# microhh/rte-rrtmgp-cpp

Measured on AMD Instinct MI355X. Metric: columns/sec (LW+SW full solve, 140 lay x 256 gpt), higher is better.
Workload: dtype f64; 1 GPU; C4 synthetic 16384 columns/GPU (16384 in total) x 140 layers x 256 g-points, LW+SW clear-sky, RCEMIP profile, synthetic k-distribution (real shapes); columns_per_gpu=16384, columns_total=16384, nlay=140, ngpt=256, flux_mode=broadband (do_broadband solvers, g-point sums on chip), columns_sorted=False, parallelism=columns sharded x1, all-gather of broadband fluxes

## Files before the change

include/rrx_hip.h:

```cpp
#ifndef RRX_HIP_H
#define RRX_HIP_H

#ifdef __cplusplus
extern "C" {
#endif

typedef signed char RrxBool;

const char* rrx_last_error(void);
int rrx_device_count(int* n);
int rrx_set_device(int dev);
int rrx_malloc(void** ptr, unsigned long long bytes);
int rrx_free(void* ptr);
int rrx_malloc_async(void** ptr, unsigned long long bytes, void* stream);
int rrx_free_async(void* ptr, void* stream);
int rrx_free_async_ordered(void* ptr, void* alloc_stream, void* release_stream);
int rrx_memcpy_h2d_stream(void* dst, const void* src, unsigned long long bytes, void* stream);
int rrx_memcpy_d2h_stream(void* dst, const void* src, unsigned long long bytes, void* stream);
int rrx_memcpy_h2d(void* dst, const void* src, unsigned long long bytes);
int rrx_memcpy_d2h(void* dst, const void* src, unsigned long long bytes);
int rrx_memcpy_d2d(void* dst, const void* src, unsigned long long bytes, void* stream);
int rrx_memset(void* dst, int value, unsigned long long bytes, void* stream);
int rrx_synchronize(void* stream);
int rrx_stream_create(void** stream);
// ... 237 lines not shown
        const F* kmajor, const F* kminor_lower, const F* kminor_upper, \
        const int* minor_limits_gpt_lower, const int* minor_limits_gpt_upper, \
        const RrxBool* minor_scales_with_density_lower, const RrxBool* minor_scales_with_density_upper, \
        const RrxBool* scale_by_complement_lower, const RrxBool* scale_by_complement_upper, \
        const int* idx_minor_lower, const int* idx_minor_upper, \
        const int* idx_minor_scaling_lower, const int* idx_minor_scaling_upper, \
        const int* kminor_start_lower, const int* kminor_start_upper, \
        const int* flavor, const F* press_ref_log, const F* temp_ref, \
        F press_ref_log_delta, F temp_ref_min, F temp_ref_delta, F press_ref_trop_log, const F* vmr_ref, \
        const F* play, const F* tlay, const F* tlev, const F* tsfc, int sfc_lay, const F* col_gas, \
        const F* pfracin, F totplnk_delta, const F* totplnk, \
        F* tau, F* pfrac, F* blay, F* blev, F* sfc_src, F* sfc_src_jac, const F* cld_tau, void* stream); \
int rrx_planck_sources_from_fractions##SFX(int ncol, int nlay, int ngpt, const int* gpoint_bands, const F* pfrac, const F* blay, \
        const F* blev, F* lay_src, F* lev_src, void* stream); \
int rrx_lw_solver_noscat_fractions##SFX( \
        int ncol, int nlay, int ngpt, RrxBool top_at_1, const F* secants, const F* weights, \
        const F* tau, const F* pfrac, const F* blay, const F* blev, const int* gpoint_bands, \
        const F* sfc_emis, const F* sfc_src, const F* inc_flux, F* flux_up_loc, F* flux_dn_loc, void* stream); \
 \
int rrx_lw_solver_noscat_fractions_byband##SFX( \
        int ncol, int nlay, int ngpt, int nbnd, RrxBool top_at_1, const F* secants, const F* weights, \
        const F* tau, const F* pfrac, const F* blay, const F* blev, const int* gpoint_bands, const int* band_lims_gpt, \
        const F* sfc_emis, const F* sfc_src, const F* inc_flux, \
        F* bnd_flux_up, F* bnd_flux_dn, F* bnd_flux_net, F* flux_up, F* flux_dn, void* stream); \
 \
int rrx_lw_solver_noscat_fractions_jac##SFX( \
        int ncol, int nlay, int ngpt, RrxBool top_at_1, const F* secants, const F* weights, \
        const F* tau, const F* pfrac, const F* blay, const F* blev, const int* gpoint_bands, \
        const F* sfc_emis, const F* sfc_src, const F* inc_flux, F* flux_up_loc, F* flux_dn_loc, \
        const F* sfc_src_jac, F* flux_up_jac, void* stream); \
 \
int rrx_lw_solver_noscat_fractions_angles##SFX( \
        int ncol, int nlay, int ngpt, RrxBool top_at_1, int nmus, const F* secants, const F* weights, \
        const F* tau, const F* pfrac, const F* blay, const F* blev, const int* gpoint_bands, \
        const F* sfc_emis, const F* sfc_src, const F* inc_flux, F* flux_up_loc, F* flux_dn_loc, \
        const F* sfc_src_jac, F* flux_up_jac, void* stream); \
 \
int rrx_lw_flux_up_adjust##SFX(int ncol, int nlev, const F* flux_up_jac, const F* t_sfc_old, const F* t_sfc_new, \
        F* flux_up, F* flux_net, void* stream); \
 \
int rrx_lw_optimal_secants##SFX(int ncol, int nlay, int ngpt, int nbnd, const int* gpoint_bands, const F* optimal_angle_fit, \
        const F* tau, F* secants, void* stream); \
 \
int rrx_lw_solver_noscat_fractions_optimal##SFX( \
        int ncol, int nlay, int ngpt, int nbnd, RrxBool top_at_1, const F* weights, \
        const F* tau, const F* pfrac, const F* blay, const F* blev, const int* gpoint_bands, const F* optimal_angle_fit, \
        const F* sfc_emis, const F* sfc_src, const F* inc_flux, F* flux_up_loc, F* flux_dn_loc, \
        const F* sfc_src_jac, F* flux_up_jac, F* secants_out, void* stream); \
 \
int rrx_lw_solver_2stream##SFX( \
        int ncol, int nlay, int ngpt, RrxBool top_at_1, \
        const F* tau, const F* ssa, const F* g, const F* lev_source, \
        const F* sfc_emis, const F* sfc_src, const F* inc_flux, \
        F* flux_up, F* flux_dn, RrxBool do_broadband, F* flux_up_loc, F* flux_dn_loc, void* stream); \
 \
int rrx_lw_solver_2stream_fractions##SFX( \
        int ncol, int nlay, int ngpt, int nbnd, RrxBool top_at_1, \
        const F* tau, const F* pfrac, const F* blev, const int* gpoint_bands, const int* band_lims_gpt, \
        const F* cld_tau, const F* cld_ssa, const F* cld_g, \
        const F* sfc_emis, const F* sfc_src, const F* inc_flux, F* flux_up, F* flux_dn, void* stream); \
 \
int rrx_lw_solver_noscat_rescaled##SFX( \
        int ncol, int nlay, int ngpt, RrxBool top_at_1, int nmus, const F* secants, const F* weights, \
        const F* tau, const F* ssa, const F* g, const F* lay_source, const F* lev_source, \
        const F* sfc_emis, const F* sfc_src, const F* inc_flux, F* flux_up, F* flux_dn, \
        RrxBool do_broadband, F* flux_up_loc, F* flux_dn_loc, RrxBool do_jacobians, const F* sfc_src_jac, F* flux_up_jac, void* stream); \
 \
int rrx_lw_solver_noscat_fractions_rescaled##SFX( \
        int ncol, int nlay, int ngpt, int nbnd, RrxBool top_at_1, const F* secants, const F* weights, \
        const F* tau, const F* pfrac, const F* blay, const F* blev, const int* gpoint_bands, const int* band_lims_gpt, \
        const F* cld_tau, const F* cld_ssa, const F* cld_g, \
        const F* sfc_emis, const F* sfc_src, const F* inc_flux, F* flux_up, F* flux_dn, void* stream); \
 \
 \
int rrx_increment_1scalar_by_1scalar##SFX(int ncol, int nlay, int ngpt, F* tau_inout, const F* tau_in, void* stream); \
int rrx_increment_2stream_by_2stream##SFX(int ncol, int nlay, int ngpt, F* tau_inout, F* ssa_inout, F* g_inout, const F* tau_in, const F* ssa_in, const F* g_in, void* stream); \
int rrx_inc_1scalar_by_1scalar_bybnd##SFX(int ncol, int nlay, int ngpt, F* tau_inout, const F* tau_in, int nbnd, const int* band_lims_gpoint, void* stream); \
int rrx_inc_2stream_by_2stream_bybnd##SFX(int ncol, int nlay, int ngpt, F* tau_inout, F* ssa_inout, F* g_inout, const F* tau_in, const F* ssa_in, const F* g_in, int nbnd, const int* band_lims_gpoint, void* stream); \
int rrx_delta_scale_2str_k##SFX(int ncol, int nlay, int ngpt, F* tau_inout, F* ssa_inout, F* g_inout, void* stream); \
 \
int rrx_sum_broadband##SFX(int ncol, int nlev, int ngpt, const F* gpt_flux, F* flux, void* stream); \
int rrx_net_broadband_precalc##SFX(int ncol, int nlev, const F* flux_dn, const F* flux_up, F* flux_net, void* stream); \
 \
int rrx_heating_rate##SFX(int ncol, int nlay, F g_over_cp, const F* flux_net, const F* plev, F* heating_rate, void* stream); \
 \
int rrx_sum_byband##SFX(int ncol, int nlev, int ngpt, int nbnd, const int* band_lims, const F* gpt_flux, F* bnd_flux, void* stream); \
int rrx_net_byband_full##SFX(int ncol, int nlev, int ngpt, int nbnd, const int* band_lims, const F* gpt_flux_dn, const F* gpt_flux_up, F* bnd_flux_net, void* stream); \
 \
int rrx_get_from_subset##SFX(int ncol, int nlay, int nbnd, int ncol_in, int col_s_in, int narr, \
        F* const* var_full, const F* const* var_sub, void* stream); \
 \
 \
int rrx_fill_gases##SFX(int ncol, int nlay, int dim1, int dim2, int ngas, int igas, F* vmr_out, const F* vmr_in, F* col_gas, const F* col_dry, void* stream); \
 \
int rrx_fill_gases_all##SFX(int ncol, int nlay, int ngas, const F* const* vmr_in, const int* dim1, const int* dim2, F* col_gas, const F* col_dry, void* stream); \
 \
int rrx_get_col_dry##SFX(int ncol, int nlay, const F* vmr_h2o, const F* plev, F* col_dry, void* stream); \
 \
int rrx_expand_and_transpose##SFX(int ncol, int nbnd, const int* band_lims_gpt, const F* arr_in, F* arr_out, void* stream); \
 \
int rrx_spread_col##SFX(int ncol, int ngpt, F* toa_src, const F* solar_source, void* stream); \
 \
int rrx_scaling_to_subset##SFX(int ncol, int ngpt, F* toa_src, const F* tsi_scaling, void* stream); \
 \
int rrx_toa_source##SFX(int ncol, int ngpt, F* toa_src, const F* solar_source, const F* tsi_scaling, void* stream); \
 \
int rrx_aerosol_optics##SFX(int ncol, int nlay, int nbnd, int nhum, int nphobic, int nphilic, const F* const* aermr, const int* aermr_per_column, \
        const F* rh, const F* plev, const F* rh_upper, const F* mext_phobic, const F* ssa_phobic, const F* g_phobic, \
        const F* mext_philic, const F* ssa_philic, const F* g_philic, F* tau, F* ssa, F* g, void* stream); \
 \
int rrx_cloud_optics_2str##SFX(int ncol, int nlay, int nbnd, int nsize_liq, int nsize_ice, \
        F radliq_lwr, F radliq_upr, F diamice_lwr, F diamice_upr, \
        const F* lut_extliq, const F* lut_ssaliq, const F* lut_asyliq, \
        const F* lut_extice, const F* lut_ssaice, const F* lut_asyice, \
        const F* clwp, const F* ciwp, const F* reliq, const F* deice, F* tau, F* ssa, F* g, void* stream); \
 \
int rrx_cloud_optics_2str_delta##SFX(int ncol, int nlay, int nbnd, int nsize_liq, int nsize_ice, \
        F radliq_lwr, F radliq_upr, F diamice_lwr, F diamice_upr, \
        const F* lut_extliq, const F* lut_ssaliq, const F* lut_asyliq, \
        const F* lut_extice, const F* lut_ssaice, const F* lut_asyice, \
        const F* clwp, const F* ciwp, const F* reliq, const F* deice, F* tau, F* ssa, F* g, void* stream); \
int rrx_cloud_optics_1scl##SFX(int ncol, int nlay, int nbnd, int nsize_liq, int nsize_ice, \
        F radliq_lwr, F radliq_upr, F diamice_lwr, F diamice_upr, \
        const F* lut_extliq, const F* lut_ssaliq, const F* lut_asyliq, \
        const F* lut_extice, const F* lut_ssaice, const F* lut_asyice, \
        const F* clwp, const F* ciwp, const F* reliq, const F* deice, F* tau, void* stream); \
 \
int rrx_subset_cols##SFX(int ncol_full, int nrest, int col_s, int ncol_sub, const F* in, F* out, void* stream); \
 \
int rrx_subset_lastdim##SFX(int n1, int ncol_full, int col_s, int ncol_sub, const F* in, F* out, void* stream); \
 \
int rrx_fill##SFX(unsigned long long n, F value, F* arr, void* stream); \
 \
int rrx_sort_columns##SFX(int ncol, const F* key, int npad, int* perm, void* stream); \
int rrx_column_spread##SFX(int ncol, const F* key, int block, F threshold, int* flag, void* stream); \
int rrx_gather_cols##SFX(int nout, unsigned long long nrest, const int* perm, int ncol_in, const F* in, F* out, void* stream); \
int rrx_scatter_cols##SFX(int n, unsigned long long nrest, const int* perm, int ncol_src, const F* in, int ncol_dst, F* out, void* stream); \
int rrx_gather_lastdim##SFX(int n1, int nout, const int* perm, const F* in, F* out, void* stream); \
 \
int rrx_sunlit_columns##SFX(int ncol, const F* mu0, const int* order, int pad_to, int* perm, int* count, void* stream); \
int rrx_scatter_cols_fill##SFX(int n, unsigned long long nrest, const int* perm, int ncol_src, const F* in, int ncol_dst, F* out, void* stream); \
 \
int rrx_mcica_increment_1scalar##SFX(int ncol, int nlay, int ngpt, int nbnd, const int* band_lims_gpt, const F* cloud_frac, const F* alpha, \
        unsigned long long seed, int domain, const int* col_id, int col_id0, F* tau_inout, const F* cld_tau, unsigned char* mask_out, void* stream); \
int rrx_mcica_increment_2stream##SFX(int ncol, int nlay, int ngpt, int nbnd, const int* band_lims_gpt, const F* cloud_frac, const F* alpha, \
        unsigned long long seed, int domain, const int* col_id, int col_id0, F* tau_inout, F* ssa_inout, F* g_inout, \
        const F* cld_tau, const F* cld_ssa, const F* cld_g, unsigned char* mask_out, void* stream); \
int rrx_mcica_cloud_mask##SFX(int ncol, int nlay, int ngpt, const F* cloud_frac, const F* alpha, unsigned long long seed, int domain, \
        const int* col_id, int col_id0, unsigned char* mask_out, void* stream); \
 \
int rrx_rt_k_null##SFX(int nx, int ny, int nz, int ngpt, int nbnd, int igpt, RrxBool top_at_1, const F* tau, const int* band_lims_gpt, \
        const F* cld_tau, F dz, int knx, int kny, int knz, F* k_null, void* stream); \
int rrx_rt_trace_counts##SFX(int nx, int ny, int nz, int ngpt, int nbnd, int igpt, RrxBool top_at_1, RrxBool independent_column, \
        const F* tau, const F* ssa, const int* band_lims_gpt, const F* cld_tau, const F* cld_ssa, const F* cld_g, \
        F dx, F dy, F dz, const F* sfc_albedo, F mu0, F azimuth, F inc_dir, F inc_dif, int knx, int kny, int knz, const F* k_null, \
        unsigned long long seed, long long photon0, long long nphotons, int max_events, \
        unsigned long long* sfc_dn_dir, unsigned long long* sfc_dn_dif, unsigned long long* sfc_up, unsigned long long* tod_up, \
        unsigned long long* abs_dir, unsigned long long* abs_dif, unsigned long long* n_capped, void* stream); \
int rrx_rt_counts_to_flux##SFX(long long n, const unsigned long long* counts, F scale, F* out, void* stream); \
int rrx_raytracer_sw##SFX(int nx, int ny, int nz, int ngpt, int nbnd, RrxBool top_at_1, RrxBool independent_column, \
        const F* tau, const F* ssa, const int* band_lims_gpt, const F* cld_tau, const F* cld_ssa, const F* cld_g, \
        F dx, F dy, F dz, const F* sfc_albedo, F mu0, F azimuth, const F* inc_dir, const F* inc_dif, int knx, int kny, int knz, \
        long long photons_per_pixel, unsigned long long seed, int max_events, \
        F* sfc_dn_dir, F* sfc_dn_dif, F* sfc_up, F* tod_up, F* abs_dir, F* abs_dif, unsigned long long* n_capped, void* stream); \
 \
int rrx_rt_bw_trace_counts##SFX(int nx, int ny, int nz, int ngpt, int nbnd, int igpt, RrxBool top_at_1, \
        const F* tau, const F* ssa, const int* band_lims_gpt, const F* cld_tau, const F* cld_ssa, const F* cld_g, \
        F dx, F dy, F dz, const F* sfc_albedo, F mu0, F azimuth, int knx, int kny, int knz, const F* k_null, \
        int sensor_type, int npx, int npy, F fov, const F* sensor, unsigned long long seed, long long ray0, long long nrays, int max_events, \
        unsigned long long* counts, unsigned long long* n_capped, unsigned long long* n_clamped, void* stream); \
int rrx_raytracer_bw##SFX(int nx, int ny, int nz, int ngpt, int nbnd, RrxBool top_at_1, \
        const F* tau, const F* ssa, const int* band_lims_gpt, const F* cld_tau, const F* cld_ssa, const F* cld_g, \
        F dx, F dy, F dz, const F* sfc_albedo, F mu0, F azimuth, const F* inc_dir, int knx, int kny, int knz, \
        int sensor_type, int npx, int npy, F fov, const F* sensor, long long rays_per_pixel, unsigned long long seed, int max_events, \
        F* radiance, unsigned long long* n_capped, unsigned long long* n_clamped, void* stream);

RRX_DECLARE(double, _f64)
RRX_DECLARE(float, _f32)

#ifdef __cplusplus
}
#endif
#endif
```

rte-rrtmgp-cpp_amd/csrc/rrx_common.h:

```cpp
#ifndef RRX_COMMON_H
#define RRX_COMMON_H

#include <hip/hip_runtime.h>
#include <cfloat>
#include <cstdlib>
#include <cmath>
#include <string>
#include <vector>
#include <stdexcept>
#include <type_traits>
#include <initializer_list>
#include <utility>
#include "rrx_hip.h"

typedef signed char Bool;

namespace rrx
{
    struct Tuning
    {
        int lw_variant = 0;
        int sw_variant = 0;
        int bb_min_groups = 512;
        int bb_gsplit = 0;
// ... 108 lines not shown
#else
    __device__ __forceinline__ float fast_rcp(const float x) { return 1.0f / x; }
#endif

    __device__ __forceinline__ double exp_neg(const double x)
    {
        const double n = __builtin_rint(x * 0x1.71547652b82fep+0);
        double r = fma(n, -0x1.62e42f0000000p-1, x);
        r = fma(n, -0x1.df473de6af279p-26, r);
        double p = 0x1.af389ecfc4b9cp-26;
        p = fma(p, r, 0x1.28917c89a43a7p-22); p = fma(p, r, 0x1.71de0db2f6b19p-19); p = fma(p, r, 0x1.a019b9149a41cp-16);
        p = fma(p, r, 0x1.a01a01a7c2efep-13); p = fma(p, r, 0x1.6c16c17889ef1p-10); p = fma(p, r, 0x1.11111111109b5p-7);
        p = fma(p, r, 0x1.5555555553d68p-5); p = fma(p, r, 0x1.5555555555556p-3); p = fma(p, r, 0x1.0000000000001p-1);
        const double t = fma(r*r, p, r);
        return __builtin_amdgcn_ldexp(t + 1.0, (int)n);
    }
    static __device__ const double exp2_64_table[64] = {
        0x1.0000000000000p+0, 0x1.02c9a3e778061p+0, 0x1.059b0d3158574p+0, 0x1.0874518759bc8p+0, 0x1.0b5586cf9890fp+0, 0x1.0e3ec32d3d1a2p+0,
        0x1.11301d0125b51p+0, 0x1.1429aaea92de0p+0, 0x1.172b83c7d517bp+0, 0x1.1a35beb6fcb75p+0, 0x1.1d4873168b9aap+0, 0x1.2063b88628cd6p+0,
        0x1.2387a6e756238p+0, 0x1.26b4565e27cddp+0, 0x1.29e9df51fdee1p+0, 0x1.2d285a6e4030bp+0, 0x1.306fe0a31b715p+0, 0x1.33c08b26416ffp+0,
        0x1.371a7373aa9cbp+0, 0x1.3a7db34e59ff7p+0, 0x1.3dea64c123422p+0, 0x1.4160a21f72e2ap+0, 0x1.44e086061892dp+0, 0x1.486a2b5c13cd0p+0,
        0x1.4bfdad5362a27p+0, 0x1.4f9b2769d2ca7p+0, 0x1.5342b569d4f82p+0, 0x1.56f4736b527dap+0, 0x1.5ab07dd485429p+0, 0x1.5e76f15ad2148p+0,
        0x1.6247eb03a5585p+0, 0x1.6623882552225p+0, 0x1.6a09e667f3bcdp+0, 0x1.6dfb23c651a2fp+0, 0x1.71f75e8ec5f74p+0, 0x1.75feb564267c9p+0,
        0x1.7a11473eb0187p+0, 0x1.7e2f336cf4e62p+0, 0x1.82589994cce13p+0, 0x1.868d99b4492edp+0, 0x1.8ace5422aa0dbp+0, 0x1.8f1ae99157736p+0,
        0x1.93737b0cdc5e5p+0, 0x1.97d829fde4e50p+0, 0x1.9c49182a3f090p+0, 0x1.a0c667b5de565p+0, 0x1.a5503b23e255dp+0, 0x1.a9e6b5579fdbfp+0,
        0x1.ae89f995ad3adp+0, 0x1.b33a2b84f15fbp+0, 0x1.b7f76f2fb5e47p+0, 0x1.bcc1e904bc1d2p+0, 0x1.c199bdd85529cp+0, 0x1.c67f12e57d14bp+0,
        0x1.cb720dcef9069p+0, 0x1.d072d4a07897cp+0, 0x1.d5818dcfba487p+0, 0x1.da9e603db3285p+0, 0x1.dfc97337b9b5fp+0, 0x1.e502ee78b3ff6p+0,
        0x1.ea4afa2a490dap+0, 0x1.efa1bee615a27p+0, 0x1.f50765b6e4540p+0, 0x1.fa7c1819e90d8p+0};
    __device__ __forceinline__ void exp_table_fill(double* lds_table)
    {
        if (threadIdx.x < 64) lds_table[threadIdx.x] = exp2_64_table[threadIdx.x];
    }
    __device__ __forceinline__ double exp_neg(const double x, const double* lds_table)
    {
        const double magic = 0x1.8p+52;
        const double t = fma(x, 0x1.71547652b82fep+6, magic);
        const double nf = t - magic;
        double r = fma(nf, -0x1.62e42fefa0000p-7, x);
        r = fma(nf, -0x1.cf79abc9e3b3ap-46, r);
        const int j = __double2loint(t) & 63;
        const int e = ((int)nf >> 6);
        const double T = lds_table[j];
        double p = 0x1.1111111111111p-7;
        p = fma(p, r, 0x1.5555555555555p-5); p = fma(p, r, 0x1.5555555555555p-3); p = fma(p, r, 0.5);
        const double q = fma(r*r, p, r);
        return __builtin_amdgcn_ldexp(fma(T, q, T), e);
    }
    __device__ __forceinline__ float exp_neg(const float x)
    {
        const float p = x * 0x1.715476p+0f;
        const float d = fmaf(x, 0x1.4ae0c0p-26f, fmaf(x, 0x1.715476p+0f, -p));
        const float y = __builtin_amdgcn_exp2f(p);
        return fmaf(y, d * 0x1.62e430p-1f, y);
    }
    __device__ __forceinline__ float exp_neg(const float x, const float*) { return exp_neg(x); }

    __device__ __forceinline__ double sqrt_pos(const double x)
    {
        const double y = __builtin_amdgcn_rsq(x);
        double g = x*y, h = 0.5*y;
        const double r = fma(-h, g, 0.5);
        g = fma(g, r, g); h = fma(h, r, h);
        const double d = fma(-g, g, x);
        return fma(d, h, g);
    }
    __device__ __forceinline__ float sqrt_pos(const float x) { return __builtin_amdgcn_sqrtf(x); }

    __device__ __forceinline__ double sqrt_nonneg(const double x)
    {
        const double y = __builtin_fmin(__builtin_amdgcn_rsq(x), 0x1p+511);
        double g = x*y, h = 0.5*y;
        const double r = fma(-h, g, 0.5);
        g = fma(g, r, g); h = fma(h, r, h);
        const double d = fma(-g, g, x);
        return fma(d, h, g);
    }
    __device__ __forceinline__ float sqrt_nonneg(const float x) { return sqrt_pos(x); }

    __device__ __forceinline__ int xcd_contiguous(const int w, const int n)
    {
        constexpr int NXCD = 8;
        const int per = n / NXCD, whole = per*NXCD;
        return (w < whole) ? (w % NXCD)*per + w / NXCD : w;
    }

    inline int ceil_div(const long long a, const long long b) { return int((a + b - 1) / b); }

    template<typename Fn> void with_flag(const bool flag, Fn&& f) { if (flag) f(std::true_type{}); else f(std::false_type{}); }

    template<int... Ks, typename Fn> bool with_k(const int need, Fn&& f)
    {
        return ((need <= Ks && (f(std::integral_constant<int,Ks>{}), true)) || ...);
    }

    inline void keep_pool_memory()
    {
        static thread_local int configured_device = -1;
        int dev = 0;
        if (hipGetDevice(&dev) != hipSuccess || dev == configured_device) return;
        hipMemPool_t pool;
        if (hipDeviceGetDefaultMemPool(&pool, dev) != hipSuccess) return;
        unsigned long long keep = ~0ull;
        if (const char* e = std::getenv("RRX_POOL_RELEASE_THRESHOLD")) keep = std::strtoull(e, nullptr, 10);
        if (hipMemPoolSetAttribute(pool, hipMemPoolAttrReleaseThreshold, &keep) == hipSuccess) configured_device = dev;
    }

    void* cached_workspace(hipStream_t st, size_t bytes);
    void release_workspace(hipStream_t st);
    void trim_workspace(hipStream_t st);
    size_t workspace_bytes(hipStream_t st);

    class WorkspaceLease
    {
        public:
            explicit WorkspaceLease(hipStream_t st) : st_(st) {}
            WorkspaceLease(const WorkspaceLease&) = delete;
            WorkspaceLease& operator=(const WorkspaceLease&) = delete;
            template<typename F> F* get(const size_t n)
            {
                if (taken_) throw std::runtime_error("workspace leased twice in one call");
                taken_ = true;
                return static_cast<F*>(cached_workspace(st_, n*sizeof(F)));
            }
            ~WorkspaceLease() { if (taken_) trim_workspace(st_); }
        private:
            hipStream_t st_;
            bool taken_ = false;
    };

    class StreamScratch
    {
        public:
            explicit StreamScratch(hipStream_t st) : st_(st) {}
            StreamScratch(const StreamScratch&) = delete;
            StreamScratch& operator=(const StreamScratch&) = delete;
            template<typename F> F* get(const size_t n, const bool zero = false)
            {
                void* p = nullptr;
                keep_pool_memory();
                if (hipMallocAsync(&p, n*sizeof(F), st_) != hipSuccess) throw std::runtime_error("workspace allocation failed");
                ptrs_.push_back(p);
                if (zero && hipMemsetAsync(p, 0, n*sizeof(F), st_) != hipSuccess) throw std::runtime_error("workspace memset failed");
                return static_cast<F*>(p);
            }
            ~StreamScratch() { for (void* p : ptrs_) (void)hipFreeAsync(p, st_); }
        private:
            hipStream_t st_;
            std::vector<void*> ptrs_;
    };
}

namespace rrx
{
    inline int broadband_gsplit(const int groups, const int ngpt, const int slots = 512)
    {
        const Tuning& t = tuning();
        if (t.bb_gsplit >= 1) return std::min(t.bb_gsplit, ngpt);
        if (t.bb_min_groups <= 1) return 1;
        int best = 1;
        double best_cost = double(ceil_div(groups, slots));
        for (int n = 2, k = 1; n <= 16 && n*4 <= ngpt; n *= 2, ++k)
        {
            const double cost = double(ceil_div((long long)groups*n, slots)) / n * (1.0 + 0.01*k);
            if (cost < best_cost) { best_cost = cost; best = n; }
        }
        return best;
// ... 154 lines not shown
```

rte-rrtmgp-cpp_amd/csrc/rrx_gas_optics.hip:

```cpp
#include <type_traits>
#include <cstdio>
#include <cstdlib>
#include "rrx_common.h"
#include "rrx_hip.h"

namespace
{
#ifndef RRX_GW_ABL
#define RRX_GW_ABL 0
#endif
template<typename F> __device__ __forceinline__ void stream_store_sbase(const char* sbase, const unsigned voff, const F v)
{
    static_assert(sizeof(F) == 4 || sizeof(F) == 8, "dword or dwordx2");
    if (RRX_GW_ABL == 7) { if (v == F(-12345.678)) *reinterpret_cast<F*>(const_cast<char*>(sbase) + voff) = v; return; }
    if constexpr (sizeof(F) == 4) asm volatile("global_store_dword %0, %1, %2 nt" :: "v"(voff), "v"(v), "s"(sbase) : "memory");
    else asm volatile("global_store_dwordx2 %0, %1, %2 nt" :: "v"(voff), "v"(v), "s"(sbase) : "memory");
}
template<typename F> __device__ __forceinline__ void stream_store(F* p, const F v)
{
    if (RRX_GW_ABL == 7) { if (v == F(-12345.678)) *p = v; return; }
    __builtin_nontemporal_store(v, p);
}

using namespace rrx;
// ... 1110 lines not shown
{
    if (const char* e = std::getenv("RRX_GW_GEOM")) return std::atoi(e) ? 1 : 0;
    return ncol >= 192 ? 1 : 0;
}
inline dim3 gather_grid(const int entries_)
{
    const int entries = entries_*GSH;
    return dim3(std::min(entries, 512));
}
inline dim3 gas_window_grid(const int geom, const int ncol, const int nlay)
{
    return geom ? dim3(ceil_div(ncol, 256), nlay) : dim3(ceil_div(ncol, 64), ceil_div(nlay, 4));
}

#ifndef RRX_GW_TIMING
#define RRX_GW_TIMING 0
#endif
#if RRX_GW_TIMING
__device__ unsigned long long g_gw_clk[8];
#define RRX_GW_T(k) { const unsigned long long t_ = __builtin_readcyclecounter(); gw_acc[k] += t_ - gw_t; gw_t = t_; }
#else
#define RRX_GW_T(k)
#endif
thread_local long long g_gw_handed = 0, g_gw_total = 0;
inline void gas_window_stats(const char* what, const int* todo, const int nblk, hipStream_t st)
{
    if (std::getenv("RRX_GW_STATS") == nullptr) return;
    int h[9];
    if (hipStreamSynchronize(st) != hipSuccess || hipMemcpy(h, todo - 8, sizeof(h), hipMemcpyDeviceToHost) != hipSuccess) return;
    g_gw_handed += h[8]; g_gw_total += nblk;
    std::fprintf(stderr, "[gas window %s] %d of %d workgroups handed back: temperature %d, pressure %d, regimes %d, chunk form %d, eta %d\n",
                 what, h[8], nblk, h[0], h[1], h[2], h[3], h[4]);
#if RRX_GW_TIMING
    unsigned long long clk[8], zero[8] = {0};
    if (hipMemcpyFromSymbol(clk, HIP_SYMBOL(g_gw_clk), sizeof(clk)) == hipSuccess)
    {
        std::fprintf(stderr, "[gas window %s] clocks per workgroup (wavefront 0): set-up %.0f, chunk prologue %.0f, staging %.0f, dma wait %.0f, barriers %.0f, g-point loop %.0f, tail %.0f, contributor scalings %.0f\n",
                     what, double(clk[0])/nblk, double(clk[1])/nblk, double(clk[2])/nblk, double(clk[3])/nblk, double(clk[4])/nblk, double(clk[5])/nblk, double(clk[6])/nblk, double(clk[7])/nblk);
        (void)hipMemcpyToSymbol(HIP_SYMBOL(g_gw_clk), zero, sizeof(zero));
    }
#endif
}

template<typename F> struct PlanckArgs
{
    const F* pfracin; const F* tlev; const F* tsfc; int sfc_lay; int nPlanckTemp; const int* gpoint_bands;
    F totplnk_delta; const F* totplnk; F* pfrac; F* blay; F* blev; F* sfc_src; F* sfc_src_jac;
};

struct GasWindowTables
{
    int ngpt, nmax, ncmax;
    static constexpr int LIT = 1 + NXW;
    __host__ __device__ int off_cinfo() const { return 2*ngpt; }
    __host__ __device__ int off_lists() const { return off_cinfo() + ncmax + 3; }
    __host__ __device__ int off_mmeta() const { return off_lists() + 2*ncmax*LIT; }
    __host__ __device__ int off_cuni()  const { return off_mmeta() + 2*MM*nmax; }
    __host__ __device__ int off_order() const { return off_cuni() + 2*ncmax; }
    static constexpr int GX = 6;
    static constexpr int RH = 12;
    static constexpr int RC = 8;
    static constexpr int REC = RH + RC*NXW;
    __host__ __device__ int off_gx()    const { return (off_order() + 2*ncmax + 3) & ~3; }
    __host__ __device__ int off_bad()   const { return off_gx() + GX*ngpt; }
    __host__ __device__ int off_rec()   const { return (off_bad() + 2*(ncmax + 1) + 3) & ~3; }
    __host__ __device__ int ints()      const { return off_rec() + 2*ncmax*REC; }
};
static_assert(GasWindowTables::REC % 4 == 0 && GasWindowTables::RH % 4 == 0 && GasWindowTables::RC == 8, "records are read as 16- and 32-byte words");
inline int gas_window_ncmax(const int ngpt, const int nband) { return (ngpt + GCH - 1) / GCH + std::max(nband, 0); }

constexpr int GW_TBL_HEADER = 8;
constexpr int GW_TBL_MAGIC = 0x52525835;
__global__ void __launch_bounds__(256)
gas_window_tables_kernel(
        const int ngpt, const int nminorlower, const int nminorupper, const int ncmax, const int nlist, const int nband,
        const int* __restrict__ gpoint_flavor,
        const int* __restrict__ flavor, const int* __restrict__ gpoint_bands, const int* __restrict__ band_lims,
        const int* __restrict__ minor_limits_gpt_lower, const int* __restrict__ minor_limits_gpt_upper,
        const Bool* __restrict__ minor_scales_with_density_lower, const Bool* __restrict__ minor_scales_with_density_upper,
        const Bool* __restrict__ scale_by_complement_lower, const Bool* __restrict__ scale_by_complement_upper,
        const int* __restrict__ idx_minor_lower, const int* __restrict__ idx_minor_upper,
        const int* __restrict__ idx_minor_scaling_lower, const int* __restrict__ idx_minor_scaling_upper,
        const int* __restrict__ kminor_start_lower, const int* __restrict__ kminor_start_upper,
        int* __restrict__ tbl)
{
    extern __shared__ int lds_int[];
    const int nmax = max(nminorlower, nminorupper);
    const GasWindowTables T{ngpt, nmax, ncmax};
    constexpr int LIT = GasWindowTables::LIT;
    int* gflav = lds_int;
    int* cinfo = lds_int + T.off_cinfo();
    int* lists = lds_int + T.off_lists();
    int* mmeta = lds_int + T.off_mmeta();
    int* cuni = lds_int + T.off_cuni();
    int* order = lds_int + T.off_order();
    int* cut = lds_int + T.off_gx();
    const int tid = threadIdx.x;
    const int ntab = T.off_gx();
    auto gx_of = [&](const int g, const int k) -> int
    {
        if (k == 0) return gpoint_bands != nullptr ? gpoint_bands[g] - 1 : -1;
        if (k == 1)
        {
            if (band_lims == nullptr) return -1;
            int b = 0;
            while (b < nband-1 && g + 1 > band_lims[2*b+1]) ++b;
            return b;
        }
        return flavor[2*gflav[((k - 2) >> 1)*ngpt + g] + (k & 1)];
    };
    for (int w = tid; w < ntab + ngpt + 4 + 2*((ngpt + 63)/64); w += 256) lds_int[w] = 0;
    __syncthreads();
    {
        for (int w = tid; w < 2*ngpt; w += 256) gflav[(w & 1)*ngpt + (w >> 1)] = gpoint_flavor[w] - 1;
        for (int w = tid; w < nminorlower; w += 256)
        {
            int* m = mmeta + MM*w;
            m[0] = idx_minor_lower[w]; m[1] = minor_scales_with_density_lower[w] ? 1 : 0;
            m[2] = idx_minor_scaling_lower[w]; m[3] = scale_by_complement_lower[w] ? 1 : 0;
            m[4] = minor_limits_gpt_lower[2*w]; m[5] = minor_limits_gpt_lower[2*w+1]; m[6] = kminor_start_lower[w];
        }
        for (int w = tid; w < nminorupper; w += 256)
        {
            int* m = mmeta + MM*(nmax + w);
            m[0] = idx_minor_upper[w]; m[1] = minor_scales_with_density_upper[w] ? 1 : 0;
            m[2] = idx_minor_scaling_upper[w]; m[3] = scale_by_complement_upper[w] ? 1 : 0;
            m[4] = minor_limits_gpt_upper[2*w]; m[5] = minor_limits_gpt_upper[2*w+1]; m[6] = kminor_start_upper[w];
        }
    }
    __syncthreads();
    {
        int* head = tbl + T.ints();
        int differs = (head[0] != GW_TBL_MAGIC || head[1] != ngpt || head[2] != nminorlower || head[3] != nminorupper
                       || head[4] != ncmax || head[5] != nlist || head[6] != nband) ? 1 : 0;
        for (int w = tid; w < 2*ngpt && !differs; w += 256) differs = (tbl[w] != gflav[w]) ? 1 : 0;
        for (int w = tid; w < 2*MM*nmax && !differs; w += 256) differs = (tbl[T.off_mmeta() + w] != mmeta[w]) ? 1 : 0;
        for (int w = tid; w < GasWindowTables::GX*ngpt && !differs; w += 256)
            differs = (tbl[T.off_gx() + w] != gx_of(w / GasWindowTables::GX, w % GasWindowTables::GX)) ? 1 : 0;
        if (!__syncthreads_or(differs)) return;
        if (tid == 0) head[0] = 0;
    }
    for (int g = tid; g < ngpt; g += 256)
        if (g > 0 && (gflav[g] != gflav[g-1] || gflav[ngpt + g] != gflav[ngpt + g-1])) cut[g] = 1;
    for (int w = tid; w < 2*nmax; w += 256)
    {
        const int r = w / nmax, i = w % nmax;
        if (i < (r == 0 ? nminorlower : nminorupper))
        {
            const int* m = mmeta + MM*w;
            const int lo = m[4]-1, hi = m[5];
            if (lo > 0 && lo < ngpt) cut[lo] = 1;
            if (hi > 0 && hi < ngpt) cut[hi] = 1;
        }
    }
    __syncthreads();
    unsigned long long* cutmask = reinterpret_cast<unsigned long long*>(cut + ((ngpt + 2) & ~1));
    for (int base = 0; base < ngpt; base += 256)
    {
        const int g = base + tid;
        const unsigned long long m = __ballot(g > 0 && g < ngpt && cut[g] != 0);
        if ((tid & 63) == 0 && base + (tid & ~63) < ngpt) cutmask[(base + tid) >> 6] = m;
    }
    __syncthreads();
    if (tid == 0)
    {
        int n = 0, start = 0;
        bool fits = true;
        auto emit_until = [&](const int p)
        {
// ... 779 lines not shown

template<typename F> size_t planck_lds_bytes(const int ngpt)
{
    return size_t(GCH)*(PL+1)*64*sizeof(F) + size_t((2*ngpt + 3) & ~3)*sizeof(int) + size_t(PL)*2*4*GCH*2*sizeof(F);
}


template<typename F>
struct GasTables
{
    int nband, ngpt, neta, npres, ntemp, nminorlower, nminorupper, idx_h2o;
    const int* gpoint_flavor; const int* band_lims_gpt;
    const F* kmajor; const F* kminor_lower; const F* kminor_upper;
    const int* minor_limits_gpt_lower; const int* minor_limits_gpt_upper;
    const Bool* minor_scales_with_density_lower; const Bool* minor_scales_with_density_upper;
    const Bool* scale_by_complement_lower; const Bool* scale_by_complement_upper;
    const int* idx_minor_lower; const int* idx_minor_upper;
    const int* idx_minor_scaling_lower; const int* idx_minor_scaling_upper;
    const int* kminor_start_lower; const int* kminor_start_upper;
    const F* krayl = nullptr;
};

template<typename F>
struct GasCells
{
    int ncol, nlay;
    const F* play; const F* tlay; const F* col_gas; const F* col_dry = nullptr; F* tau = nullptr; F* ssa = nullptr; F* g = nullptr;
    const Bool* tropo = nullptr; const F* col_mix = nullptr; const F* fmajor = nullptr; const F* fminor = nullptr;
    const int* jeta = nullptr; const int* jtemp = nullptr; const int* jpress = nullptr;
};

struct TodoTail { const int* todo = nullptr; int gx = 1, nblk = 1, nz = 1, geom = 0; };

inline size_t gather_lds_bytes(const int ngpt, const int nminorlower, const int nminorupper)
{
    const int nchunk = (ngpt + GCH - 1) / GCH, nmax = std::max(nminorlower, nminorupper);
    const size_t lds = (size_t(3)*ngpt + size_t(2)*nchunk*(1 + ITEM*nmax) + size_t(2)*MM*nmax)*sizeof(int);
    if (lds > 64*1024) throw std::runtime_error("minor-gas index exceeds 64 KiB of LDS");
    return lds;
}

template<typename F, int MODE, bool DIRECT, bool CLD>
void launch_tau_absorption(hipStream_t st, const dim3 grid, const size_t lds, const GasTables<F>& k, const GasCells<F>& c, const InterpArgs<F>& ia,
                           const TodoTail& t = TodoTail())
{
    tau_absorption_kernel<F,MODE,DIRECT,CLD><<<grid, dim3(64, 4), lds, st>>>(
            c.ncol, c.nlay, k.ngpt, k.neta, k.npres, k.ntemp, k.nminorlower, k.nminorupper, k.idx_h2o, k.gpoint_flavor,
            k.kmajor, k.kminor_lower, k.kminor_upper, k.minor_limits_gpt_lower, k.minor_limits_gpt_upper,
            k.minor_scales_with_density_lower, k.minor_scales_with_density_upper,
            k.scale_by_complement_lower, k.scale_by_complement_upper,
            k.idx_minor_lower, k.idx_minor_upper, k.idx_minor_scaling_lower, k.idx_minor_scaling_upper,
            k.kminor_start_lower, k.kminor_start_upper,
            c.tropo, c.col_mix, c.fmajor, c.fminor, c.play, c.tlay, c.col_gas, c.col_dry, c.jeta, c.jtemp, c.jpress, k.krayl,
            c.tau, c.ssa, c.g, ia, t.todo, t.gx, t.nblk, t.nz, t.geom);
}

struct GasWindowPlan
{
    bool windowed = false;
    int geom = 0, nblk = 0, nz = 1, ncmax = 0;
    dim3 grid;
    size_t lds = 0;
    int* todo = nullptr; int* tbl = nullptr;
    TodoTail tail() const { return windowed ? TodoTail{todo, int(grid.x), nblk, nz, geom} : TodoTail(); }
};

template<typename F>
GasWindowPlan gas_window_plan(hipStream_t st, StreamScratch& scratch, const GasTables<F>& k, const GasCells<F>& c, const InterpArgs<F>& ia,
                              const int mode, const bool pf, const int nlist, const int* gpoint_bands)
{
    GasWindowPlan p;
    const int nchunk = (k.ngpt + GCH - 1) / GCH;
    const int nmax = std::max(k.nminorlower, k.nminorupper);
    p.ncmax = gas_window_ncmax(k.ngpt, k.nband);
    p.lds = gas_window_lds_bytes<F>(k.ngpt, nmax, p.ncmax, mode, pf);
    p.windowed = tuning().go_window && p.lds <= 64*1024 && size_t(c.ncol)*c.nlay*sizeof(F) < (size_t(1) << 32)
                 && size_t(k.ngpt)*k.ntemp*k.neta*(k.npres+1)*sizeof(F) < (size_t(1) << 32);
    if (!p.windowed) return p;
    p.geom = gas_window_geometry(c.ncol);
    p.grid = gas_window_grid(p.geom, c.ncol, c.nlay);
    p.nblk = int(p.grid.x)*int(p.grid.y);
    p.nz = gas_window_parts(p.nblk, nchunk);
    p.todo = scratch.get<int>(size_t(9) + size_t(p.nblk)*p.nz) + 8;
    if (hipMemsetAsync(p.todo - 8, 0, 9*sizeof(int), st) != hipSuccess) throw std::runtime_error("memset failed");
    const GasWindowTables T{k.ngpt, nmax, p.ncmax};
    const int* lims = ia.cld_tau != nullptr ? ia.cld_lims : nullptr;
    p.tbl = gas_window_tables(st, k.gpoint_flavor, k.ngpt, k.nminorlower, k.nminorupper, p.ncmax, nlist, (pf ? 1 : 0) + (lims != nullptr ? 2 : 0));
    gas_window_tables_kernel<<<1, 256, size_t(T.off_gx() + k.ngpt + 4 + 2*((k.ngpt + 63)/64))*sizeof(int), st>>>(
            k.ngpt, k.nminorlower, k.nminorupper, p.ncmax, nlist, k.nband, k.gpoint_flavor, ia.flavor, gpoint_bands, lims,
            k.minor_limits_gpt_lower, k.minor_limits_gpt_upper,
            k.minor_scales_with_density_lower, k.minor_scales_with_density_upper, k.scale_by_complement_lower, k.scale_by_complement_upper,
            k.idx_minor_lower, k.idx_minor_upper, k.idx_minor_scaling_lower, k.idx_minor_scaling_upper,
            k.kminor_start_lower, k.kminor_start_upper, p.tbl);
    return p;
}

template<typename F, int MODE, bool PF, bool CLD>
void launch_gas_window(hipStream_t st, const GasWindowPlan& p, const GasTables<F>& k, const GasCells<F>& c, const InterpArgs<F>& ia,
                       const PlanckArgs<F>& pa = PlanckArgs<F>())
{
    gas_window_kernel<F,MODE,PF,CLD><<<dim3(p.grid.x, p.grid.y, p.nz), dim3(64, 4), p.lds, st>>>(
            c.ncol, c.nlay, k.ngpt, k.neta, k.npres, k.ntemp, k.nminorlower, k.nminorupper, k.idx_h2o, k.gpoint_flavor,
            k.kmajor, k.kminor_lower, k.kminor_upper, k.minor_limits_gpt_lower, k.minor_limits_gpt_upper,
            k.minor_scales_with_density_lower, k.minor_scales_with_density_upper,
            k.scale_by_complement_lower, k.scale_by_complement_upper,
            k.idx_minor_lower, k.idx_minor_upper, k.idx_minor_scaling_lower, k.idx_minor_scaling_upper,
            k.kminor_start_lower, k.kminor_start_upper, c.play, c.tlay, c.col_gas, c.col_dry, k.krayl, ia,
            c.tau, c.ssa, c.g, pa, p.todo, p.geom, p.tbl, p.ncmax);
}

template<bool ALLOWED, typename F, typename Fn>
void with_cld(const InterpArgs<F>& ia, Fn&& fn)
{
    if constexpr (ALLOWED) { if (ia.cld_tau != nullptr) { fn(std::bool_constant<true>{}); return; } }
    fn(std::bool_constant<false>{});
}

template<typename F>
int gas_optics_lw_fractions_impl(const GasTables<F>& k, const GasCells<F>& c, const InterpArgs<F>& ia, const PlanckArgs<F>& pa, void* stream)
{
    RRX_TRY
    if (c.ncol <= 0 || c.nlay <= 0 || k.ngpt <= 0) throw std::runtime_error("empty problem");
    hipStream_t st = static_cast<hipStream_t>(stream);
    const size_t lds = gather_lds_bytes(k.ngpt, k.nminorlower, k.nminorupper);
    StreamScratch scratch(st);
    const GasWindowPlan p = gas_window_plan<F>(st, scratch, k, c, ia, 2, true, NXW, pa.gpoint_bands);
    const dim3 g2 = p.windowed ? gather_grid(p.nblk*p.nz) : dim3(ceil_div(c.ncol, 64), ceil_div(c.nlay, 4));
    const TodoTail t = p.tail();
    with_cld<true>(ia, [&](auto CLD_)
    {
        constexpr bool CLD = decltype(CLD_)::value;
        if (p.windowed)
        {
            launch_gas_window<F,2,true,CLD>(st, p, k, c, ia, pa);
            gas_window_stats("lw + fractions", p.todo, p.nblk*p.nz, st);
        }
        launch_tau_absorption<F,2,true,CLD>(st, g2, lds, k, c, ia, t);
    });
    planck_fraction_kernel<F><<<g2, dim3(64, 4), size_t(2)*k.ngpt*sizeof(int), st>>>(
            c.ncol, c.nlay, k.ngpt, k.neta, k.npres, k.ntemp, pa.nPlanckTemp, c.play, c.tlay, pa.tlev, pa.tsfc, pa.sfc_lay, c.col_gas, ia,
            pa.gpoint_bands, pa.pfracin, pa.totplnk_delta, pa.totplnk, k.gpoint_flavor, pa.pfrac, pa.blay, pa.blev, pa.sfc_src, pa.sfc_src_jac,
            t.todo, t.gx, t.nblk, t.nz, t.geom);
    RRX_CATCH("rrx_gas_optics_lw_fractions")
}

template<typename F, int MODE, bool DIRECT = false>
int tau_absorption_impl(const GasTables<F>& k, const GasCells<F>& c, void* stream, const char* name, const InterpArgs<F>& ia = InterpArgs<F>())
{
    RRX_TRY
    if (c.ncol <= 0 || c.nlay <= 0 || k.ngpt <= 0) throw std::runtime_error("empty problem");
    hipStream_t st = static_cast<hipStream_t>(stream);
    const size_t lds = gather_lds_bytes(k.ngpt, k.nminorlower, k.nminorupper);
    constexpr bool HAS_CLD = DIRECT && MODE != 0;
    StreamScratch scratch(st);
    GasWindowPlan p;
    if constexpr (DIRECT && MODE != 0) p = gas_window_plan<F>(st, scratch, k, c, ia, MODE, false, (MODE == 1) ? NCW : NXW, nullptr);
    with_cld<HAS_CLD>(ia, [&](auto CLD_)
    {
        constexpr bool CLD = decltype(CLD_)::value;
        if constexpr (DIRECT && MODE != 0)
        {
            if (p.windowed)
            {
                launch_gas_window<F,MODE,false,CLD>(st, p, k, c, ia);
                gas_window_stats(MODE == 1 ? "sw" : "lw", p.todo, p.nblk*p.nz, st);
                launch_tau_absorption<F,MODE,DIRECT,CLD>(st, gather_grid(p.nblk*p.nz), lds, k, c, ia, p.tail());
                return;
            }
        }
        launch_tau_absorption<F,MODE,DIRECT,CLD>(st, dim3(ceil_div(c.ncol, 64), ceil_div(c.nlay, 4)), lds, k, c, ia);
    });
    RRX_CATCH(name)
}
}


// ... 332 lines not shown
```

rte-rrtmgp-cpp_amd/csrc/rrx_misc.hip:

```cpp
#include <mutex>
#include <vector>
#include <cstdlib>
#include <initializer_list>
#include "rrx_common.h"
#include "rrx_hip.h"

namespace rrx
{
    static thread_local std::string g_last_error;
    void set_error(const std::string& msg) { g_last_error = msg; }
    Tuning& tuning()
    {
        static thread_local Tuning t = []
        {
            Tuning d;
            if (const char* e = getenv("RRX_SYNC")) d.sync_waves = atoi(e);
            if (const char* e = getenv("RRX_GO_SHARE")) d.go_share = atoi(e);
            if (const char* e = getenv("RRX_GO_WINDOW")) d.go_window = atoi(e);
            return d;
        }();
        return t;
    }
    namespace
    {
// ... 90 lines not shown
{
    RRX_GRID_STRIDE(i, n) tau1[i] = tau1[i] + tau2[i];
}

template<typename F>
__device__ __forceinline__ void inc_2str(F& tau1, F& ssa1, F& g1, const F tau2, const F ssa2, const F g2, const F eps)
{
    const F tau12 = tau1 + tau2;
    const F tauscat12 = (tau1 * ssa1) + (tau2 * ssa2);
    g1 = ((tau1 * ssa1 * g1) + (tau2 * ssa2 * g2)) / max(tauscat12, eps);
    ssa1 = tauscat12 / max(eps, tau12);
    tau1 = tau12;
}

template<typename F>
__global__ void inc_2str_kernel(const size_t n, const F eps, F* __restrict__ tau1, F* __restrict__ ssa1, F* __restrict__ g1,
        const F* __restrict__ tau2, const F* __restrict__ ssa2, const F* __restrict__ g2)
{
    RRX_GRID_STRIDE(i, n)
    {
        F t = tau1[i], w = ssa1[i], gg = g1[i];
        inc_2str(t, w, gg, tau2[i], ssa2[i], g2[i], eps);
        tau1[i] = t; ssa1[i] = w; g1[i] = gg;
    }
}

template<typename F>
__global__ void inc_1scl_bybnd_kernel(const size_t ncl, F* __restrict__ tau1, const F* __restrict__ tau2,
        const int nbnd, const int* __restrict__ band_lims_gpt)
{
    const int igpt = blockIdx.y;
    for (int ibnd=0; ibnd<nbnd; ++ibnd)
        if (igpt+1 >= band_lims_gpt[2*ibnd] && igpt+1 <= band_lims_gpt[2*ibnd+1])
        {
            RRX_GRID_STRIDE(i, ncl) tau1[i + igpt*ncl] = tau1[i + igpt*ncl] + tau2[i + ibnd*ncl];
        }
}

template<typename F>
__global__ void inc_2str_bybnd_kernel(const size_t ncl, const F eps, F* __restrict__ tau1, F* __restrict__ ssa1, F* __restrict__ g1,
        const F* __restrict__ tau2, const F* __restrict__ ssa2, const F* __restrict__ g2,
        const int nbnd, const int* __restrict__ band_lims_gpt)
{
    const int igpt = blockIdx.y;
    for (int ibnd=0; ibnd<nbnd; ++ibnd)
        if (igpt+1 >= band_lims_gpt[2*ibnd] && igpt+1 <= band_lims_gpt[2*ibnd+1])
        {
            RRX_GRID_STRIDE(i, ncl)
            {
                const size_t o = i + igpt*ncl, b = i + ibnd*ncl;
                F t = tau1[o], w = ssa1[o], gg = g1[o];
                inc_2str(t, w, gg, tau2[b], ssa2[b], g2[b], eps);
                tau1[o] = t; ssa1[o] = w; g1[o] = gg;
            }
        }
}

template<typename F>
__global__ void delta_scale_kernel(const size_t n, const F eps, F* __restrict__ tau, F* __restrict__ ssa, F* __restrict__ g)
{
    RRX_GRID_STRIDE(i, n)
    {
        const F gv = g[i], wv = ssa[i];
        const F f = gv * gv;
        const F wf = wv * f;
        tau[i] *= (F(1.) - wf);
        ssa[i] = (wv - wf) / max(eps, F(1.) - wf);
        g[i] = (gv - f) / max(eps, F(1.) - f);
    }
}

template<typename F>
__global__ void sum_broadband_kernel(const size_t nlc, const int ngpt, const F* __restrict__ in, F* __restrict__ out)
{
    RRX_GRID_STRIDE(i, nlc)
    {
        F s = F(0.);
        for (int ig=0; ig<ngpt; ++ig) s += in[i + size_t(ig)*nlc];
        out[i] = s;
    }
}

template<typename F>
__global__ void net_kernel(const size_t n, const F* __restrict__ dn, const F* __restrict__ up, F* __restrict__ net)
{
    RRX_GRID_STRIDE(i, n) net[i] = dn[i] - up[i];
}

template<typename F, bool NET>
__global__ void byband_kernel(const size_t nlc, const int* __restrict__ band_lims, const F* __restrict__ a, const F* __restrict__ b, F* __restrict__ out)
{
    const int ibnd = blockIdx.y;
    const int g0 = band_lims[2*ibnd]-1, g1 = band_lims[2*ibnd+1]-1;
    if (g1 < g0)
    {
        RRX_GRID_STRIDE(i, nlc) out[i + size_t(ibnd)*nlc] = F(0.);
        return;
    }
    RRX_GRID_STRIDE(i, nlc)
    {
        F s = NET ? a[i + size_t(g0)*nlc] - b[i + size_t(g0)*nlc] : a[i + size_t(g0)*nlc];
        for (int ig=g0+1; ig<=g1; ++ig)
            s += NET ? a[i + size_t(ig)*nlc] - b[i + size_t(ig)*nlc] : a[i + size_t(ig)*nlc];
        out[i + size_t(ibnd)*nlc] = s;
    }
}

template<typename F> struct PtrPack { F* full[4]; const F* sub[4]; };

template<typename F>
__global__ void get_from_subset_kernel(const int ncol, const size_t nrest, const int ncol_in, const int col_s_in, const int narr, const PtrPack<F> p)
{
    const size_t n = size_t(ncol_in)*nrest;
    RRX_GRID_STRIDE(i, n)
    {
        const size_t ic = i % ncol_in, r = i / ncol_in;
        const size_t o = ic + col_s_in - 1 + r*ncol;
        for (int a=0; a<narr; ++a) p.full[a][o] = p.sub[a][i];
    }
}

template<typename F>
__global__ void fill_gases_kernel(const int ncol, const int nlay, const int dim1, const int dim2, const int igas,
        F* __restrict__ vmr_out, const F* __restrict__ vmr_in, F* __restrict__ col_gas, const F* __restrict__ col_dry)
{
    const size_t ncl = size_t(ncol)*nlay;
    RRX_GRID_STRIDE(i, ncl)
    {
        if (igas > 0)
        {
            F v;
            if (dim1 == 1 && dim2 == 1) v = vmr_in[0];
            else if (dim1 == 1)         v = vmr_in[i / ncol];
            else                        v = vmr_in[i];
            vmr_out[i + size_t(igas-1)*ncl] = v;
            col_gas[i + size_t(igas)*ncl] = v * col_dry[i];
        }
        else
            col_gas[i] = col_dry[i];
    }
}

constexpr int RRX_MAX_GASES = 32;
template<typename F> struct GasTable { const F* vmr[RRX_MAX_GASES]; int dim1[RRX_MAX_GASES], dim2[RRX_MAX_GASES]; };

template<typename F>
__global__ void fill_gases_all_kernel(const int ncol, const int nlay, const int ngas, const GasTable<F> gt,
                                      F* __restrict__ col_gas, const F* __restrict__ col_dry)
{
    const size_t ncl = size_t(ncol)*nlay;
    RRX_GRID_STRIDE(i, ncl)
    {
        const F cd = col_dry[i];
        col_gas[i] = cd;
        for (int igas=0; igas<ngas; ++igas)
        {
            const F* __restrict__ src = gt.vmr[igas];
            const F v = (gt.dim1[igas] == 1 && gt.dim2[igas] == 1) ? src[0] : (gt.dim1[igas] == 1 ? src[i / ncol] : src[i]);
            col_gas[i + size_t(igas+1)*ncl] = v * cd;
        }
    }
}

template<typename F>
__global__ void col_dry_kernel(const int ncol, const int nlay, const F* __restrict__ vmr_h2o, const F* __restrict__ plev, F* __restrict__ col_dry)
{
    constexpr F g0 = 9.80665;
    constexpr F avogad = 6.02214076e23;
    constexpr F m_dry = 0.028964;
    constexpr F m_h2o = 0.018016;
    const size_t ncl = size_t(ncol)*nlay;
    RRX_GRID_STRIDE(i, ncl)
    {
        const F delta_plev = abs(plev[i] - plev[i + ncol]);
        const F h = vmr_h2o[i];
        const F m_air = (m_dry + m_h2o * h) / (F(1.) + h);
        F cd = F(10.) * delta_plev * avogad / (F(1000.)*m_air*F(100.)*g0);
        cd /= (F(1.) + h);
        col_dry[i] = cd;
    }
}

template<typename F>
__global__ void expand_and_transpose_kernel(const int ncol, const int nbnd, const int* __restrict__ limits, const F* __restrict__ in, F* __restrict__ out)
{
    const int ibnd = blockIdx.y;
    const int g0 = limits[2*ibnd]-1, g1 = limits[2*ibnd+1];
    RRX_GRID_STRIDE(icol, size_t(ncol))
    {
        const F v = in[ibnd + icol*nbnd];
        for (int ig=g0; ig<g1; ++ig) out[icol + size_t(ig)*ncol] = v;
    }
}

template<typename F>
__global__ void spread_col_kernel(const int ncol, const int ngpt, F* __restrict__ out, const F* __restrict__ src)
{
    const F v = src[blockIdx.y];
    for (int icol = blockIdx.x*blockDim.x + threadIdx.x; icol < ncol; icol += gridDim.x*blockDim.x) out[icol + size_t(blockIdx.y)*ncol] = v;
}

template<typename F>
__global__ void scale_cols_kernel(const int ncol, const int ngpt, F* __restrict__ out, const F* __restrict__ fac)
{
    for (int icol = blockIdx.x*blockDim.x + threadIdx.x; icol < ncol; icol += gridDim.x*blockDim.x) out[icol + size_t(blockIdx.y)*ncol] *= fac[icol];
}

template<typename F>
__global__ void toa_source_kernel(const int ncol, const int ngpt, F* __restrict__ out, const F* __restrict__ src, const F* __restrict__ fac)
{
    const F v = src[blockIdx.y];
    for (int icol = blockIdx.x*blockDim.x + threadIdx.x; icol < ncol; icol += gridDim.x*blockDim.x) out[icol + size_t(blockIdx.y)*ncol] = v * fac[icol];
}

template<typename F>
__device__ __forceinline__ void cloud_from_table(const F cwp, const F re, const int nsteps, const F step_size, const F offset,
        const F* __restrict__ tau_table, const F* __restrict__ ssa_table, const F* __restrict__ asy_table,
        F& tau, F& taussa, F& taussag)
{
    if (cwp > F(0.))
    {
        const int index = min(int((re - offset) / step_size)+1, nsteps-1);
        const F fint = (re - offset) / step_size - (index-1);
        tau = cwp * (tau_table[index-1] + fint * (tau_table[index] - tau_table[index-1]));
        taussa = tau * (ssa_table[index-1] + fint * (ssa_table[index] - ssa_table[index-1]));
        taussag = taussa * (asy_table[index-1] + fint * (asy_table[index] - asy_table[index-1]));
    }
    else { tau = F(0.); taussa = F(0.); taussag = F(0.); }
}

template<typename F, bool TWOSTR, bool DELTA>
__global__ void cloud_optics_kernel(const size_t ncl, const int nbnd, const int nsize_liq, const int nsize_ice,
        const F radliq_lwr, const F liq_step, const F diamice_lwr, const F ice_step,
        const F* __restrict__ lut_extliq, const F* __restrict__ lut_ssaliq, const F* __restrict__ lut_asyliq,
        const F* __restrict__ lut_extice, const F* __restrict__ lut_ssaice, const F* __restrict__ lut_asyice,
        const F* __restrict__ clwp, const F* __restrict__ ciwp, const F* __restrict__ reliq, const F* __restrict__ deice,
        F* __restrict__ tau, F* __restrict__ ssa, F* __restrict__ g)
{
    const F eps = Lim<F>::eps();
    const F eps_delta = Lim<F>::tiny()*F(3.);
    RRX_GRID_STRIDE(i, ncl)
    {
        const F lw = clwp[i], iw = ciwp[i], rl = reliq[i], di = deice[i];
        int il = 1, ii = 1; F fl = F(0.), fi = F(0.);
        if (lw > F(0.)) { il = min(int((rl - radliq_lwr) / liq_step)+1, nsize_liq-1); fl = (rl - radliq_lwr) / liq_step - (il-1); }
        if (iw > F(0.)) { ii = min(int((di - diamice_lwr) / ice_step)+1, nsize_ice-1); fi = (di - diamice_lwr) / ice_step - (ii-1); }
        for (int ibnd=0; ibnd<nbnd; ++ibnd)
        {
            F lt = F(0.), lts = F(0.), ltsg = F(0.), it = F(0.), its = F(0.), itsg = F(0.);
            if (lw > F(0.))
            {
                const F* te = lut_extliq + size_t(ibnd)*nsize_liq; const F* ts = lut_ssaliq + size_t(ibnd)*nsize_liq; const F* ta = lut_asyliq + size_t(ibnd)*nsize_liq;
                lt = lw * (te[il-1] + fl * (te[il] - te[il-1]));
                lts = lt * (ts[il-1] + fl * (ts[il] - ts[il-1]));
                ltsg = lts * (ta[il-1] + fl * (ta[il] - ta[il-1]));
            }
            if (iw > F(0.))
            {
                const F* te = lut_extice + size_t(ibnd)*nsize_ice; const F* ts = lut_ssaice + size_t(ibnd)*nsize_ice; const F* ta = lut_asyice + size_t(ibnd)*nsize_ice;
                it = iw * (te[ii-1] + fi * (te[ii] - te[ii-1]));
                its = it * (ts[ii-1] + fi * (ts[ii] - ts[ii-1]));
                itsg = its * (ta[ii-1] + fi * (ta[ii] - ta[ii-1]));
            }
            const size_t o = i + size_t(ibnd)*ncl;
            if constexpr (TWOSTR)
            {
                const F t = lt + it, tsc = lts + its, tsg = ltsg + itsg;
                F tv = t, wv = tsc / max(t, eps), gv = tsg / max(tsc, eps);
                if constexpr (DELTA)
                {
                    const F f = gv * gv;
                    const F wf = wv * f;
                    tv *= (F(1.) - wf);
                    const F w2 = (wv - wf) / max(eps_delta, F(1.) - wf);
                    gv = (gv - f) / max(eps_delta, F(1.) - f);
                    wv = w2;
                }
                tau[o] = tv; ssa[o] = wv; g[o] = gv;
            }
            else
                tau[o] = (lt - lts) + (it - its);
        }
    }
}

template<typename F> struct AerosolSpecies { const F* mmr[11]; int per_column[11]; };

__constant__ const signed char aerosol_species_table[11][3] = {
    {0, 1, 0}, {1, 1, 1}, {2, 1, 2},
    {3, 0, 0}, {4, 0, 7}, {5, 0, 5},
    {7, 0, 9}, {6, 1, 3},
    {8, 0, 10}, {9, 0, 10},
    {10, 1, 4}};

template<typename F>
// ... 111 lines not shown
        hipEvent_t ev;
        ok = hipEventCreateWithFlags(&ev, hipEventDisableTiming) == hipSuccess;
        if (ok)
        {
            ok = hipEventRecord(ev, a) == hipSuccess && hipStreamWaitEvent(r, ev, 0) == hipSuccess;
            (void)hipEventDestroy(ev);
        }
    }
    if (ok && hipFreeAsync(ptr, r) == hipSuccess) return 0;
    (void)hipGetLastError();
    RRX_HIP_OK(hipFree(ptr), "rrx_free_async_ordered");
    return 0;
}
int rrx_memcpy_h2d_stream(void* dst, const void* src, unsigned long long bytes, void* stream)
{
    RRX_HIP_OK(hipMemcpyAsync(dst, src, bytes, hipMemcpyHostToDevice, static_cast<hipStream_t>(stream)), "rrx_memcpy_h2d_stream");
    RRX_HIP_OK(hipStreamSynchronize(static_cast<hipStream_t>(stream)), "rrx_memcpy_h2d_stream");
    return 0;
}
int rrx_memcpy_d2h_stream(void* dst, const void* src, unsigned long long bytes, void* stream)
{
    RRX_HIP_OK(hipMemcpyAsync(dst, src, bytes, hipMemcpyDeviceToHost, static_cast<hipStream_t>(stream)), "rrx_memcpy_d2h_stream");
    RRX_HIP_OK(hipStreamSynchronize(static_cast<hipStream_t>(stream)), "rrx_memcpy_d2h_stream");
    return 0;
}
int rrx_memcpy_h2d(void* dst, const void* src, unsigned long long bytes) { RRX_HIP_OK(hipMemcpy(dst, src, bytes, hipMemcpyHostToDevice), "rrx_memcpy_h2d"); return 0; }
int rrx_memcpy_d2h(void* dst, const void* src, unsigned long long bytes) { RRX_HIP_OK(hipMemcpy(dst, src, bytes, hipMemcpyDeviceToHost), "rrx_memcpy_d2h"); return 0; }
int rrx_memcpy_d2d(void* dst, const void* src, unsigned long long bytes, void* stream) { RRX_HIP_OK(hipMemcpyAsync(dst, src, bytes, hipMemcpyDeviceToDevice, static_cast<hipStream_t>(stream)), "rrx_memcpy_d2d"); return 0; }
int rrx_memset(void* dst, int value, unsigned long long bytes, void* stream) { RRX_HIP_OK(hipMemsetAsync(dst, value, bytes, static_cast<hipStream_t>(stream)), "rrx_memset"); return 0; }
int rrx_synchronize(void* stream) { RRX_HIP_OK(hipStreamSynchronize(static_cast<hipStream_t>(stream)), "rrx_synchronize"); return 0; }
int rrx_stream_create(void** stream) { hipStream_t s; RRX_HIP_OK(hipStreamCreate(&s), "rrx_stream_create"); *stream = s; return 0; }
int rrx_stream_destroy(void* stream)
{
    rrx::release_workspace(static_cast<hipStream_t>(stream));
    RRX_HIP_OK(hipStreamDestroy(static_cast<hipStream_t>(stream)), "rrx_stream_destroy");
    return 0;
}
int rrx_release_workspace(void* stream) { rrx::release_workspace(static_cast<hipStream_t>(stream)); return 0; }
unsigned long long rrx_workspace_bytes(void* stream) { return rrx::workspace_bytes(static_cast<hipStream_t>(stream)); }

#define ST static_cast<hipStream_t>(stream)

int rrx_subset_nd(void* out, const void* in, int elem_bytes, int ndim, const int* sub_dims, const long long* strides,
                  const int* starts, const int* spread, void* stream)
{
    RRX_TRY
    if (ndim < 1 || ndim > 7) throw std::runtime_error("ndim must be 1..7");
    if (elem_bytes != 1 && elem_bytes != 4 && elem_bytes != 8) throw std::runtime_error("element size must be 1, 4 or 8 bytes");
    SubsetND sd; sd.ndim = ndim; size_t n = 1;
    for (int d=0; d<ndim; ++d)
    {
        if (sub_dims[d] < 0) throw std::runtime_error("negative extent");
        sd.sub_dims[d] = sub_dims[d]; sd.strides[d] = strides[d]; sd.starts[d] = starts[d]; sd.spread[d] = spread[d]; n *= size_t(sub_dims[d]);
    }
    if (n == 0) return 0;
    if (elem_bytes == 8) subset_nd_kernel<double><<<grid1d(n), 256, 0, ST>>>(sd, n, static_cast<const double*>(in), static_cast<double*>(out));
    else if (elem_bytes == 4) subset_nd_kernel<int><<<grid1d(n), 256, 0, ST>>>(sd, n, static_cast<const int*>(in), static_cast<int*>(out));
    else subset_nd_kernel<signed char><<<grid1d(n), 256, 0, ST>>>(sd, n, static_cast<const signed char*>(in), static_cast<signed char*>(out));
    RRX_CATCH("rrx_subset_nd")
}

#define RRX_DEFINE_MISC(F, SFX) \
int rrx_increment_1scalar_by_1scalar##SFX(int ncol, int nlay, int ngpt, F* tau_inout, const F* tau_in, void* stream) \
{ RRX_TRY const size_t n = size_t(ncol)*nlay*ngpt; \
  inc_1scl_kernel<F><<<grid1d(n), 256, 0, ST>>>(n, tau_inout, tau_in); RRX_CATCH("rrx_increment_1scalar_by_1scalar") } \
int rrx_increment_2stream_by_2stream##SFX(int ncol, int nlay, int ngpt, F* tau_inout, F* ssa_inout, F* g_inout, const F* tau_in, const F* ssa_in, const F* g_in, void* stream) \
{ RRX_TRY const size_t n = size_t(ncol)*nlay*ngpt; \
  inc_2str_kernel<F><<<grid1d(n), 256, 0, ST>>>(n, rrx::Lim<F>::tiny()*F(3.), tau_inout, ssa_inout, g_inout, tau_in, ssa_in, g_in); RRX_CATCH("rrx_increment_2stream_by_2stream") } \
int rrx_inc_1scalar_by_1scalar_bybnd##SFX(int ncol, int nlay, int ngpt, F* tau_inout, const F* tau_in, int nbnd, const int* band_lims_gpoint, void* stream) \
{ RRX_TRY const size_t ncl = extent({ncol, nlay}); if (extent({ngpt, nbnd}) == 0 || ncl == 0) return 0; \
  inc_1scl_bybnd_kernel<F><<<dim3(std::min(grid1d(ncl), 1024), ngpt), 256, 0, ST>>>(ncl, tau_inout, tau_in, nbnd, band_lims_gpoint); RRX_CATCH("rrx_inc_1scalar_by_1scalar_bybnd") } \
int rrx_inc_2stream_by_2stream_bybnd##SFX(int ncol, int nlay, int ngpt, F* tau_inout, F* ssa_inout, F* g_inout, const F* tau_in, const F* ssa_in, const F* g_in, int nbnd, const int* band_lims_gpoint, void* stream) \
{ RRX_TRY const size_t ncl = extent({ncol, nlay}); if (extent({ngpt, nbnd}) == 0 || ncl == 0) return 0; \
  inc_2str_bybnd_kernel<F><<<dim3(std::min(grid1d(ncl), 1024), ngpt), 256, 0, ST>>>(ncl, rrx::Lim<F>::tiny()*F(3.), tau_inout, ssa_inout, g_inout, tau_in, ssa_in, g_in, nbnd, band_lims_gpoint); RRX_CATCH("rrx_inc_2stream_by_2stream_bybnd") } \
int rrx_delta_scale_2str_k##SFX(int ncol, int nlay, int ngpt, F* tau_inout, F* ssa_inout, F* g_inout, void* stream) \
{ RRX_TRY const size_t n = size_t(ncol)*nlay*ngpt; \
  delta_scale_kernel<F><<<grid1d(n), 256, 0, ST>>>(n, rrx::Lim<F>::tiny()*F(3.), tau_inout, ssa_inout, g_inout); RRX_CATCH("rrx_delta_scale_2str_k") } \
int rrx_sum_broadband##SFX(int ncol, int nlev, int ngpt, const F* gpt_flux, F* flux, void* stream) \
{ RRX_TRY const size_t n = size_t(ncol)*nlev; \
  sum_broadband_kernel<F><<<grid1d(n), 256, 0, ST>>>(n, ngpt, gpt_flux, flux); RRX_CATCH("rrx_sum_broadband") } \
int rrx_net_broadband_precalc##SFX(int ncol, int nlev, const F* flux_dn, const F* flux_up, F* flux_net, void* stream) \
{ RRX_TRY const size_t n = size_t(ncol)*nlev; \
  net_kernel<F><<<grid1d(n), 256, 0, ST>>>(n, flux_dn, flux_up, flux_net); RRX_CATCH("rrx_net_broadband_precalc") } \
int rrx_heating_rate##SFX(int ncol, int nlay, F g_over_cp, const F* flux_net, const F* plev, F* heating_rate, void* stream) \
{ RRX_TRY const size_t n = extent({ncol, nlay}); if (n == 0) return 0; \
  heating_rate_kernel<F><<<grid1d(n), 256, 0, ST>>>(n, ncol, g_over_cp, flux_net, plev, heating_rate); RRX_CATCH("rrx_heating_rate") } \
int rrx_sum_byband##SFX(int ncol, int nlev, int ngpt, int nbnd, const int* band_lims, const F* gpt_flux, F* bnd_flux, void* stream) \
{ RRX_TRY (void)ngpt; const size_t n = extent({ncol, nlev}); if (n == 0 || extent({nbnd}) == 0) return 0; \
  byband_kernel<F,false><<<dim3(std::min(grid1d(n), 1024), nbnd), 256, 0, ST>>>(n, band_lims, gpt_flux, (const F*)nullptr, bnd_flux); RRX_CATCH("rrx_sum_byband") } \
int rrx_net_byband_full##SFX(int ncol, int nlev, int ngpt, int nbnd, const int* band_lims, const F* gpt_flux_dn, const F* gpt_flux_up, F* bnd_flux_net, void* stream) \
{ RRX_TRY (void)ngpt; const size_t n = extent({ncol, nlev}); if (n == 0 || extent({nbnd}) == 0) return 0; \
  byband_kernel<F,true><<<dim3(std::min(grid1d(n), 1024), nbnd), 256, 0, ST>>>(n, band_lims, gpt_flux_dn, gpt_flux_up, bnd_flux_net); RRX_CATCH("rrx_net_byband_full") } \
int rrx_get_from_subset##SFX(int ncol, int nlay, int nbnd, int ncol_in, int col_s_in, int narr, F* const* var_full, const F* const* var_sub, void* stream) \
{ RRX_TRY if (narr < 1 || narr > 4) throw std::runtime_error("narr must be 1..4"); \
  if (col_s_in < 1 || col_s_in - 1 + ncol_in > ncol) throw std::runtime_error("column range outside the full array"); \
  PtrPack<F> p; for (int a=0; a<narr; ++a) { p.full[a] = var_full[a]; p.sub[a] = var_sub[a]; } \
  const size_t nrest = extent({nlay, nbnd}); if (extent({ncol_in}) == 0 || nrest == 0) return 0; \
  get_from_subset_kernel<F><<<grid1d(size_t(ncol_in)*nrest), 256, 0, ST>>>(ncol, nrest, ncol_in, col_s_in, narr, p); RRX_CATCH("rrx_get_from_subset") } \
int rrx_fill_gases##SFX(int ncol, int nlay, int dim1, int dim2, int ngas, int igas, F* vmr_out, const F* vmr_in, F* col_gas, const F* col_dry, void* stream) \
{ RRX_TRY (void)ngas; if (extent({ncol, nlay}) == 0) return 0; \
  fill_gases_kernel<F><<<grid1d(size_t(ncol)*nlay), 256, 0, ST>>>(ncol, nlay, dim1, dim2, igas, vmr_out, vmr_in, col_gas, col_dry); RRX_CATCH("rrx_fill_gases") } \
int rrx_fill_gases_all##SFX(int ncol, int nlay, int ngas, const F* const* vmr_in, const int* dim1, const int* dim2, F* col_gas, const F* col_dry, void* stream) \
{ RRX_TRY if (ngas < 0 || ngas > RRX_MAX_GASES) throw std::runtime_error("more gases than rrx_fill_gases_all takes"); \
  if (extent({ncol, nlay}) == 0) return 0; \
  GasTable<F> gt; for (int i=0; i<ngas; ++i) { gt.vmr[i] = vmr_in[i]; gt.dim1[i] = dim1[i]; gt.dim2[i] = dim2[i]; } \
  fill_gases_all_kernel<F><<<grid1d(size_t(ncol)*nlay), 256, 0, ST>>>(ncol, nlay, ngas, gt, col_gas, col_dry); RRX_CATCH("rrx_fill_gases_all") } \
int rrx_get_col_dry##SFX(int ncol, int nlay, const F* vmr_h2o, const F* plev, F* col_dry, void* stream) \
{ RRX_TRY col_dry_kernel<F><<<grid1d(size_t(ncol)*nlay), 256, 0, ST>>>(ncol, nlay, vmr_h2o, plev, col_dry); RRX_CATCH("rrx_get_col_dry") } \
int rrx_expand_and_transpose##SFX(int ncol, int nbnd, const int* band_lims_gpt, const F* arr_in, F* arr_out, void* stream) \
{ RRX_TRY if (extent({ncol, nbnd}) == 0) return 0; \
  expand_and_transpose_kernel<F><<<dim3(std::min(grid1d(ncol), 1024), nbnd), 256, 0, ST>>>(ncol, nbnd, band_lims_gpt, arr_in, arr_out); RRX_CATCH("rrx_expand_and_transpose") } \
int rrx_spread_col##SFX(int ncol, int ngpt, F* toa_src, const F* solar_source, void* stream) \
{ RRX_TRY spread_col_kernel<F><<<dim3(std::min(ceil_div(ncol, 256), 64), ngpt), 256, 0, ST>>>(ncol, ngpt, toa_src, solar_source); RRX_CATCH("rrx_spread_col") } \
int rrx_scaling_to_subset##SFX(int ncol, int ngpt, F* toa_src, const F* tsi_scaling, void* stream) \
{ RRX_TRY scale_cols_kernel<F><<<dim3(std::min(ceil_div(ncol, 256), 64), ngpt), 256, 0, ST>>>(ncol, ngpt, toa_src, tsi_scaling); RRX_CATCH("rrx_scaling_to_subset") } \
int rrx_toa_source##SFX(int ncol, int ngpt, F* toa_src, const F* solar_source, const F* tsi_scaling, void* stream) \
{ RRX_TRY if (ncol <= 0 || ngpt <= 0) throw std::runtime_error("empty problem"); \
  if (tsi_scaling == nullptr) spread_col_kernel<F><<<dim3(std::min(ceil_div(ncol, 256), 64), ngpt), 256, 0, ST>>>(ncol, ngpt, toa_src, solar_source); \
  else toa_source_kernel<F><<<dim3(std::min(ceil_div(ncol, 256), 64), ngpt), 256, 0, ST>>>(ncol, ngpt, toa_src, solar_source, tsi_scaling); RRX_CATCH("rrx_toa_source") } \
int rrx_aerosol_optics##SFX(int ncol, int nlay, int nbnd, int nhum, int nphobic, int nphilic, const F* const* aermr, const int* aermr_per_column, \
        const F* rh, const F* plev, const F* rh_upper, const F* mext_phobic, const F* ssa_phobic, const F* g_phobic, \
        const F* mext_philic, const F* ssa_philic, const F* g_philic, F* tau, F* ssa, F* g, void* stream) \
{ RRX_TRY if (nphobic < 11 || nphilic < 5) throw std::runtime_error("aerosol tables need >= 11 hydrophobic and >= 5 hydrophilic species"); \
  if (nhum < 1) throw std::runtime_error("no humidity classes"); \
  AerosolSpecies<F> sp; for (int a=0; a<11; ++a) { if (!aermr[a]) throw std::runtime_error("missing aerosol mixing ratio"); sp.mmr[a] = aermr[a]; sp.per_column[a] = aermr_per_column ? aermr_per_column[a] : 1; } \
  aerosol_optics_kernel<F><<<grid1d(size_t(ncol)*nlay), 256, 0, ST>>>(ncol, nlay, nbnd, nhum, sp, rh, plev, rh_upper, \
      mext_phobic, ssa_phobic, g_phobic, mext_philic, ssa_philic, g_philic, tau, ssa, g); RRX_CATCH("rrx_aerosol_optics") } \
int rrx_cloud_optics_2str##SFX(int ncol, int nlay, int nbnd, int nsize_liq, int nsize_ice, \
        F radliq_lwr, F radliq_upr, F diamice_lwr, F diamice_upr, \
        const F* lut_extliq, const F* lut_ssaliq, const F* lut_asyliq, const F* lut_extice, const F* lut_ssaice, const F* lut_asyice, \
        const F* clwp, const F* ciwp, const F* reliq, const F* deice, F* tau, F* ssa, F* g, void* stream) \
{ RRX_TRY const size_t ncl = size_t(ncol)*nlay; \
  cloud_optics_kernel<F,true,false><<<grid1d(ncl), 256, 0, ST>>>(ncl, nbnd, nsize_liq, nsize_ice, \
      radliq_lwr, (radliq_upr - radliq_lwr)/(nsize_liq - F(1.)), diamice_lwr, (diamice_upr - diamice_lwr)/(nsize_ice - F(1.)), \
      lut_extliq, lut_ssaliq, lut_asyliq, lut_extice, lut_ssaice, lut_asyice, clwp, ciwp, reliq, deice, tau, ssa, g); RRX_CATCH("rrx_cloud_optics_2str") } \
int rrx_cloud_optics_2str_delta##SFX(int ncol, int nlay, int nbnd, int nsize_liq, int nsize_ice, \
        F radliq_lwr, F radliq_upr, F diamice_lwr, F diamice_upr, \
        const F* lut_extliq, const F* lut_ssaliq, const F* lut_asyliq, const F* lut_extice, const F* lut_ssaice, const F* lut_asyice, \
        const F* clwp, const F* ciwp, const F* reliq, const F* deice, F* tau, F* ssa, F* g, void* stream) \
{ RRX_TRY const size_t ncl = size_t(ncol)*nlay; \
  cloud_optics_kernel<F,true,true><<<grid1d(ncl), 256, 0, ST>>>(ncl, nbnd, nsize_liq, nsize_ice, \
      radliq_lwr, (radliq_upr - radliq_lwr)/(nsize_liq - F(1.)), diamice_lwr, (diamice_upr - diamice_lwr)/(nsize_ice - F(1.)), \
      lut_extliq, lut_ssaliq, lut_asyliq, lut_extice, lut_ssaice, lut_asyice, clwp, ciwp, reliq, deice, tau, ssa, g); RRX_CATCH("rrx_cloud_optics_2str_delta") } \
int rrx_cloud_optics_1scl##SFX(int ncol, int nlay, int nbnd, int nsize_liq, int nsize_ice, \
        F radliq_lwr, F radliq_upr, F diamice_lwr, F diamice_upr, \
        const F* lut_extliq, const F* lut_ssaliq, const F* lut_asyliq, const F* lut_extice, const F* lut_ssaice, const F* lut_asyice, \
        const F* clwp, const F* ciwp, const F* reliq, const F* deice, F* tau, void* stream) \
{ RRX_TRY const size_t ncl = size_t(ncol)*nlay; \
  cloud_optics_kernel<F,false,false><<<grid1d(ncl), 256, 0, ST>>>(ncl, nbnd, nsize_liq, nsize_ice, \
      radliq_lwr, (radliq_upr - radliq_lwr)/(nsize_liq - F(1.)), diamice_lwr, (diamice_upr - diamice_lwr)/(nsize_ice - F(1.)), \
      lut_extliq, lut_ssaliq, lut_asyliq, lut_extice, lut_ssaice, lut_asyice, clwp, ciwp, reliq, deice, tau, (F*)nullptr, (F*)nullptr); RRX_CATCH("rrx_cloud_optics_1scl") } \
int rrx_subset_cols##SFX(int ncol_full, int nrest, int col_s, int ncol_sub, const F* in, F* out, void* stream) \
{ RRX_TRY const size_t n = extent({ncol_sub, nrest}); \
  if (col_s < 1 || col_s - 1 + ncol_sub > ncol_full) throw std::runtime_error("column range outside the full array"); \
  if (n == 0) return 0; \
  subset_cols_kernel<F><<<grid1d(size_t(ncol_sub)*nrest), 256, 0, ST>>>(ncol_full, size_t(nrest), col_s, ncol_sub, in, out); RRX_CATCH("rrx_subset_cols") } \
int rrx_subset_lastdim##SFX(int n1, int ncol_full, int col_s, int ncol_sub, const F* in, F* out, void* stream) \
{ RRX_TRY const size_t n = extent({n1, ncol_sub}); \
  if (col_s < 1 || col_s - 1 + ncol_sub > ncol_full) throw std::runtime_error("column range outside the full array"); \
  if (n == 0) return 0; \
  if (hipMemcpyAsync(out, in + size_t(col_s-1)*n1, n*sizeof(F), hipMemcpyDeviceToDevice, ST) != hipSuccess) \
      throw std::runtime_error("hipMemcpyAsync failed"); RRX_CATCH("rrx_subset_lastdim") } \
int rrx_fill##SFX(unsigned long long n, F value, F* arr, void* stream) \
{ RRX_TRY if (n == 0) return 0; \
  fill_kernel<F><<<grid1d(n), 256, 0, ST>>>(n, value, arr); RRX_CATCH("rrx_fill") }

// ... 4 lines not shown
```

rte-rrtmgp-cpp_amd/csrc/rrx_solver_lw.hip:

```cpp
#include "rrx_common.h"
#include "rrx_hip.h"

#pragma clang fp contract(fast)

namespace
{
using namespace rrx;

constexpr int CL = 8;
constexpr int LL = 8;

template<typename F, int V, int K, bool JAC, bool ACC>
__global__ void __launch_bounds__(256, 2)
lw_noscat_scan_kernel(
        const int ncol, const int nlay, const int ngpt, const int top_at_1, const int imu,
        const F* __restrict__ secants, const F* __restrict__ weights,
        const F* __restrict__ tau, const F* __restrict__ lay_source, const F* __restrict__ lev_source,
        const F* __restrict__ sfc_emis, const F* __restrict__ sfc_src, const F* __restrict__ inc_flux,
        F* __restrict__ flux_up, F* __restrict__ flux_dn,
        const F* __restrict__ sfc_src_jac, F* __restrict__ flux_up_jac, const int sync_waves)
{
    constexpr int W = 2;
    const int lane = threadIdx.x & 63;
    const int wave = threadIdx.x >> 6;
// ... 606 lines not shown

template<typename F, bool JAC, bool ACC>
__global__ void __launch_bounds__(256)
lw_noscat_serial_kernel(
        const int ncol, const int nlay, const int ngpt, const int top_at_1, const int imu,
        const F* __restrict__ secants, const F* __restrict__ weights,
        const F* __restrict__ tau, const F* __restrict__ lay_source, const F* __restrict__ lev_source,
        const F* __restrict__ sfc_emis, const F* __restrict__ sfc_src, const F* __restrict__ inc_flux,
        F* __restrict__ flux_up, F* __restrict__ flux_dn,
        const F* __restrict__ sfc_src_jac, F* __restrict__ flux_up_jac)
{
    const int icol = blockIdx.x*blockDim.x + threadIdx.x;
    const int igpt = blockIdx.y;
    if (icol >= ncol) return;

    const int nlev = nlay+1;
    const size_t ncl = size_t(ncol);
    const size_t lay_base = size_t(igpt)*ncl*nlay + icol;
    const size_t lev_base = size_t(igpt)*ncl*nlev + icol;
    const size_t sfc_idx = size_t(igpt)*ncl + icol;
    const F pi = F(3.14159265358979323846);
    const F tau_thres = sqrt(sqrt(Lim<F>::eps()));
    const F D = secants[sfc_idx + size_t(imu)*ncl*ngpt];
    const F scale = pi * weights[imu];

    auto layer = [&](const int s, F& trans, F& s_dn, F& s_up)
    {
        const int ml = top_at_1 ? s : nlay-1-s;
        const int m_above = top_at_1 ? ml : ml+1;
        const int m_below = top_at_1 ? ml+1 : ml;
        const F tau_loc = tau[lay_base + size_t(ml)*ncl] * D;
        const F ls = lay_source[lay_base + size_t(ml)*ncl];
        const F lev_above = lev_source[lev_base + size_t(m_above)*ncl];
        const F lev_below = lev_source[lev_base + size_t(m_below)*ncl];
        trans = exp(-tau_loc);
        const F fact = tau_loc > tau_thres ?
            (F(1.) - trans) / tau_loc - trans :
            tau_loc * (F(.5) + tau_loc * (F(-1./3.) + tau_loc * F(1./8.)));
        s_dn = (F(1.) - trans) * lev_below + F(2.) * fact * (ls - lev_below);
        s_up = (F(1.) - trans) * lev_above + F(2.) * fact * (ls - lev_above);
    };
    auto put = [&](F* arr, const int t, const F val)
    {
        const int ml = top_at_1 ? t : nlay - t;
        const size_t o = lev_base + size_t(ml)*ncl;
        arr[o] = ACC ? arr[o] + scale*val : scale*val;
    };

    F dn = (inc_flux != nullptr) ? inc_flux[sfc_idx] / pi : F(0.);
    for (int s=0; s<nlay; ++s)
    {
        F trans, s_dn, s_up;
        layer(s, trans, s_dn, s_up);
        put(flux_dn, s, dn);
        dn = trans*dn + s_dn;
    }
    put(flux_dn, nlay, dn);

    const F emis = sfc_emis[sfc_idx];
    F up = dn * (F(1.) - emis) + emis * sfc_src[sfc_idx];
    F jc = JAC ? emis * sfc_src_jac[sfc_idx] : F(0.);
    put(flux_up, nlay, up);
    if constexpr (JAC) put(flux_up_jac, nlay, jc);
    for (int s=nlay-1; s>=0; --s)
    {
        F trans, s_dn, s_up;
        layer(s, trans, s_dn, s_up);
        up = trans*up + s_up;
        put(flux_up, s, up);
        if constexpr (JAC) { jc = trans*jc; put(flux_up_jac, s, jc); }
    }
}


template<typename F>
__global__ void lw_secants_array_kernel(
        const int ncol, const int ngpt, const int n_gauss_quad, const int max_gauss_pts,
        const F* __restrict__ gauss_Ds, F* __restrict__ secants)
{
    const size_t n = size_t(ncol)*ngpt*n_gauss_quad;
    for (size_t i = size_t(blockIdx.x)*blockDim.x + threadIdx.x; i < n; i += size_t(gridDim.x)*blockDim.x)
    {
        const int imu = int(i / (size_t(ncol)*ngpt));
        secants[i] = gauss_Ds[imu + (n_gauss_quad-1)*max_gauss_pts];
    }
}


template<typename F>
__global__ void __launch_bounds__(256)
lw_optimal_secants_kernel(
        const int ncol, const int nlay, const int* __restrict__ gpoint_bands, const F* __restrict__ fit,
        const F* __restrict__ tau, F* __restrict__ secants)
{
    const int icol = blockIdx.x*blockDim.x + threadIdx.x;
    const int igpt = blockIdx.y;
    if (icol >= ncol) return;
    const size_t ncl = size_t(ncol);
    const F* __restrict__ t = tau + size_t(igpt)*ncl*nlay + icol;
    F s = F(0.);
    #pragma unroll 8
    for (int ilay=0; ilay<nlay; ++ilay) s += t[size_t(ilay)*ncl];
    const int ib = gpoint_bands[igpt] - 1;
    secants[size_t(igpt)*ncl + icol] = fit[2*ib] * exp(-s) + fit[2*ib+1];
}

template<typename F>
int lw_optimal_secants_impl(const int ncol, const int nlay, const int ngpt, const int nbnd, const int* gpoint_bands,
                            const F* optimal_angle_fit, const F* tau, F* secants, void* stream)
{
    const char* entry = "rrx_lw_optimal_secants";
    const char* bad = nullptr;
    if (ncol <= 0) bad = "ncol must be positive";
    else if (nlay <= 0) bad = "nlay must be positive";
    else if (ngpt <= 0 || ngpt > 65535) bad = "ngpt must be 1..65535";
    else if (nbnd <= 0) bad = "nbnd must be positive";
    else if (gpoint_bands == nullptr) bad = "gpoint_bands is null";
    else if (optimal_angle_fit == nullptr) bad = "optimal_angle_fit is null";
    else if (tau == nullptr) bad = "tau is null";
    else if (secants == nullptr) bad = "secants is null";
    if (bad != nullptr) { set_error(std::string(entry) + ": " + bad); return 1; }
    RRX_TRY
    lw_optimal_secants_kernel<F><<<dim3(ceil_div(ncol, 256), ngpt), 256, 0, static_cast<hipStream_t>(stream)>>>(
            ncol, nlay, gpoint_bands, optimal_angle_fit, tau, secants);
    RRX_CATCH(entry)
}

template<typename F, int V>
bool launch_scan(
        hipStream_t st, const bool jac, const bool acc,
        const int ncol, const int nlay, const int ngpt, const int top_at_1, const int imu,
        const F* secants, const F* weights, const F* tau, const F* lay_source, const F* lev_source,
        const F* sfc_emis, const F* sfc_src, const F* inc_flux, F* flux_up, F* flux_dn,
        const F* sfc_src_jac, F* flux_up_jac)
{
    const dim3 grid(ceil_div(ncol, 2*CL*V), ngpt);
    const int sync_waves = tuning().sync_waves;
    return with_k<2, 4, 6, 9, 12, 17>(ceil_div(nlay+1, 2*LL), [&](auto kk)
    {
        with_flag(jac, [&](auto j) { with_flag(acc, [&](auto a)
        {
            lw_noscat_scan_kernel<F,V,decltype(kk)::value,decltype(j)::value,decltype(a)::value><<<grid, 256, 0, st>>>(
                ncol, nlay, ngpt, top_at_1, imu, secants, weights, tau, lay_source, lev_source,
                sfc_emis, sfc_src, inc_flux, flux_up, flux_dn, sfc_src_jac, flux_up_jac, sync_waves);
        }); });
    });
}

template<typename F>
struct BbArgs
{
    int ncol, nlay, ngpt, top_at_1;
    const F *secants, *weights, *tau, *lay_source , *lev_source, *blay, *blev;
    const int* gpoint_bands;
    const F *sfc_emis, *sfc_src, *inc_flux;
    F *flux_up, *flux_dn;
    const F* sfc_src_jac = nullptr; F* flux_up_jac = nullptr;
    int nmus = 1;
    const F* opt_fit = nullptr; F* secants_out = nullptr;
    const int* band_lims = nullptr; int nbnd = 0;
};

template<typename F, int V, int W, int CLT, bool LITE, int NW, bool JAC, bool MU, bool OPT = false>
bool launch_bb2(hipStream_t st, const BbArgs<F>& a)
{
    static_assert(!MU || LITE, "several angles: Planck-lite inputs only");
    static_assert(!OPT || (LITE && !MU), "optimal angles: Planck-lite inputs, one angle");
// ... 471 lines not shown
```

rte-rrtmgp-cpp_amd/hip_kernels.py:

```python
import ctypes
import os
import numpy as np
import torch

from ._ffi import Lib, PtrArg, HEADER_PATH

_HERE = os.path.dirname(os.path.abspath(__file__))
LIB_PATH = os.path.join(_HERE, "lib", "librrx_hip.so")


def load_library():
    if not os.path.exists(LIB_PATH):
        raise RuntimeError(
            f"{LIB_PATH} is missing: build it with `python -c 'import __graft_entry__ as g; g.build()'` "
            "(hipcc --offload-arch=gfx950). The product path has no CPU fallback.")
    return ctypes.CDLL(LIB_PATH)


class HipKernels:
    name = "hip"

    def __init__(self, dtype=np.float64, device="cuda:0", stream=None):
        if not torch.cuda.is_available():
            raise RuntimeError("HipKernels needs a GPU (no CPU fallback on the product path)")
# ... 503 lines not shown
    def rt_trace_counts(self, tau, ssa, igpt, nx, ny, dx, dy, dz, sfc_albedo, mu0, azimuth, inc_dir, inc_dif, kn_grid, k_null, seed,
                        photon0, nphotons, top_at_1=False, independent_column=False, cloud=None, band_lims=None, counts=None,
                        max_events=None):
        dims, (lims, ct, cw, cg) = self._rt_scene(tau, nx, ny, cloud, band_lims)
        knx, kny, knz = (int(k) for k in kn_grid)
        counts = self.rt_zero_counts(dims[2], dims[0]*dims[1]) if counts is None else counts
        self._c("rt_trace_counts", *dims, igpt, top_at_1, independent_column, tau, ssa, lims, ct, cw, cg, dx, dy, dz, sfc_albedo, mu0, azimuth,
                inc_dir, inc_dif, knx, kny, knz, k_null, int(seed) & 0xFFFFFFFFFFFFFFFF, photon0, nphotons,
                self.RT_MAX_EVENTS if max_events is None else max_events, *(counts[k] for k in self.RT_COUNTS), counts["n_capped"])
        return counts

    def rt_counts_to_flux(self, counts, scale, out):
        self._c("rt_counts_to_flux", counts.numel(), counts, scale, out)
        return out

    def raytracer_sw(self, tau, ssa, nx, ny, dx, dy, dz, sfc_albedo, mu0, azimuth, inc_dir, inc_dif, kn_grid, photons_per_pixel, seed,
                     top_at_1=False, independent_column=False, cloud=None, band_lims=None, max_events=None):
        dims, (lims, ct, cw, cg) = self._rt_scene(tau, nx, ny, cloud, band_lims)
        nz, ngpt, ncol = dims[2], dims[3], dims[0]*dims[1]
        knx, kny, knz = (int(k) for k in kn_grid)
        inc_dir = np.ascontiguousarray(np.asarray(inc_dir, dtype=self.np_dtype).reshape(-1))
        inc_dif = np.ascontiguousarray(np.asarray(inc_dif, dtype=self.np_dtype).reshape(-1))
        if inc_dir.size != ngpt or inc_dif.size != ngpt:
            raise ValueError("raytracer: inc_dir, inc_dif are (ngpt,)")
        out = {k: self.empty((ncol,)) for k in self.RT_COUNTS[:4]}
        out.update({k: self.empty((nz, ncol)) for k in self.RT_COUNTS[4:]})
        n_capped = torch.zeros((1,), dtype=torch.int64, device=self.device)
        self._c("raytracer_sw", *dims, top_at_1, independent_column, tau, ssa, lims, ct, cw, cg, dx, dy, dz, sfc_albedo, mu0, azimuth, inc_dir,
                inc_dif, knx, kny, knz, photons_per_pixel, int(seed) & 0xFFFFFFFFFFFFFFFF,
                self.RT_MAX_EVENTS if max_events is None else max_events, *(out[k] for k in self.RT_COUNTS), n_capped)
        out["n_capped"] = int(n_capped.item())
        return out

    def _rt_sensor(self, camera):
        numbers = np.concatenate([np.asarray(v, dtype=np.float64).reshape(3) for v in (camera.position, camera.e_w, camera.e_h, camera.e_d)])
        return (int(camera.type), int(camera.npx), int(camera.npy), camera.fov, np.ascontiguousarray(numbers.astype(self.np_dtype)))

    def rt_bw_zero_counts(self, npix):
        return {k: torch.zeros((n,), dtype=torch.int64, device=self.device) for k, n in (("counts", npix), ("n_capped", 1), ("n_clamped", 1))}

    def rt_bw_trace_counts(self, tau, ssa, igpt, nx, ny, dx, dy, dz, sfc_albedo, mu0, azimuth, kn_grid, k_null, camera, seed, ray0, nrays,
                           top_at_1=False, cloud=None, band_lims=None, counts=None, max_events=None):
        dims, (lims, ct, cw, cg) = self._rt_scene(tau, nx, ny, cloud, band_lims)
        knx, kny, knz = (int(k) for k in kn_grid)
        sensor = self._rt_sensor(camera)
        counts = self.rt_bw_zero_counts(sensor[1]*sensor[2]) if counts is None else counts
        self._c("rt_bw_trace_counts", *dims, igpt, top_at_1, tau, ssa, lims, ct, cw, cg, dx, dy, dz, sfc_albedo, mu0, azimuth, knx, kny, knz,
                k_null, *sensor, int(seed) & 0xFFFFFFFFFFFFFFFF, ray0, nrays, self.RT_MAX_EVENTS if max_events is None else max_events,
                counts["counts"], counts["n_capped"], counts["n_clamped"])
        return counts

    def raytracer_bw(self, tau, ssa, nx, ny, dx, dy, dz, sfc_albedo, mu0, azimuth, inc_dir, kn_grid, camera, rays_per_pixel, seed,
                     top_at_1=False, cloud=None, band_lims=None, max_events=None):
        dims, (lims, ct, cw, cg) = self._rt_scene(tau, nx, ny, cloud, band_lims)
        knx, kny, knz = (int(k) for k in kn_grid)
        inc_dir = np.ascontiguousarray(np.asarray(inc_dir, dtype=self.np_dtype).reshape(-1))
        if inc_dir.size != dims[3]:
            raise ValueError("raytracer: inc_dir is (ngpt,)")
        sensor = self._rt_sensor(camera)
        radiance = self.empty((sensor[2], sensor[1]))
        n_capped = torch.zeros((1,), dtype=torch.int64, device=self.device)
        n_clamped = torch.zeros((1,), dtype=torch.int64, device=self.device)
        self._c("raytracer_bw", *dims, top_at_1, tau, ssa, lims, ct, cw, cg, dx, dy, dz, sfc_albedo, mu0, azimuth, inc_dir, knx, kny, knz,
                *sensor, rays_per_pixel, int(seed) & 0xFFFFFFFFFFFFFFFF, self.RT_MAX_EVENTS if max_events is None else max_events,
                radiance, n_capped, n_clamped)
        return dict(radiance=radiance, n_capped=int(n_capped.item()), n_clamped=int(n_clamped.item()))

    def delta_scale_2str_k(self, tau, ssa, g):
        ngpt, nlay, ncol = tau.shape
        self._c("delta_scale_2str_k", ncol, nlay, ngpt, tau, ssa, g)

    def sum_broadband(self, gpt_flux, out=None):
        ngpt, nlev, ncol = gpt_flux.shape
        out = self.empty((nlev, ncol)) if out is None else out
        self._c("sum_broadband", ncol, nlev, ngpt, gpt_flux, out)
        return out

    def net_broadband_precalc(self, flux_dn, flux_up, out=None):
        nlev, ncol = flux_dn.shape
        out = self.empty((nlev, ncol)) if out is None else out
        self._c("net_broadband_precalc", ncol, nlev, flux_dn, flux_up, out)
        return out

    def heating_rate(self, flux_net, plev, g_over_cp=9.80665/1004.64):
        nlev, ncol = flux_net.shape
        out = self.empty((nlev-1, ncol))
        self._c("heating_rate", ncol, nlev-1, g_over_cp, flux_net, plev, out)
        return out

    def sum_byband(self, gpt_flux, band_lims):
        ngpt, nlev, ncol = gpt_flux.shape
        nbnd = band_lims.shape[0]
        out = self.empty((nbnd, nlev, ncol))
        self._c("sum_byband", ncol, nlev, ngpt, nbnd, band_lims, gpt_flux, out)
        return out

    def net_byband_full(self, gpt_dn, gpt_up, band_lims):
        ngpt, nlev, ncol = gpt_dn.shape
        nbnd = band_lims.shape[0]
        out = self.empty((nbnd, nlev, ncol))
        self._c("net_byband_full", ncol, nlev, ngpt, nbnd, band_lims, gpt_dn, gpt_up, out)
        return out

    def get_col_dry(self, vmr_h2o, plev, out=None):
        nlay, ncol = vmr_h2o.shape
        out = self.empty((nlay, ncol)) if out is None else out
        self._c("get_col_dry", ncol, nlay, vmr_h2o, plev, out)
        return out

    @staticmethod
    def _vmr_dims(name, v, nlay, ncol):
        shape = tuple(v.shape)
        if v.numel() == 1:
            return 1, 1
        if shape in ((nlay,), (nlay, 1)):
            return 1, nlay
        if shape == (nlay, ncol):
            return ncol, nlay
        raise ValueError(f"fill_gases: {name} has shape {shape}; expected a scalar, a profile ({nlay},) or ({nlay}, 1), "
                         f"or a field ({nlay}, {ncol})")

    def fill_gases(self, kd, vmr_by_name, col_dry):
        nlay, ncol = col_dry.shape
        col_gas = self.empty((kd.ngas+1, nlay, ncol))
        vs = [vmr_by_name[name] for name in kd.gas_names]
        dims = [self._vmr_dims(name, v, nlay, ncol) for name, v in zip(kd.gas_names, vs)]
        if len(vs) <= 32:
            self._c("fill_gases_all", ncol, nlay, len(vs), (ctypes.c_void_p * len(vs))(*[v.data_ptr() for v in vs]),
                    (ctypes.c_int * len(vs))(*[d[0] for d in dims]), (ctypes.c_int * len(vs))(*[d[1] for d in dims]), col_gas, col_dry)
            return col_gas
        vmr = self.empty((kd.ngas, nlay, ncol))
        self._c("fill_gases", ncol, nlay, ncol, nlay, kd.ngas, 0, vmr, col_dry, col_gas, col_dry)
        for i, (v, (d1, d2)) in enumerate(zip(vs, dims), start=1):
            self._c("fill_gases", ncol, nlay, d1, d2, kd.ngas, i, vmr, v, col_gas, col_dry)
        return col_gas

    def expand_and_transpose(self, band_lims, arr_in, ngpt, out=None):
        ncol, nbnd = arr_in.shape
        out = self.empty((ngpt, ncol)) if out is None else out
        self._c("expand_and_transpose", ncol, nbnd, band_lims, arr_in, out)
        return out

    def spread_col(self, ncol, solar_source):
        out = self.empty((solar_source.shape[0], ncol))
        self._c("spread_col", ncol, solar_source.shape[0], out, solar_source)
        return out

    def toa_source(self, ncol, solar_source, tsi_scaling):
        out = self.empty((solar_source.shape[0], ncol))
        self._c("toa_source", ncol, solar_source.shape[0], out, solar_source, tsi_scaling)
        return out

    def scaling_to_subset(self, toa_src, tsi_scaling):
        ngpt, ncol = toa_src.shape
        self._c("scaling_to_subset", ncol, ngpt, toa_src, tsi_scaling)

    def cloud_optics_2str(self, lut, clwp, ciwp, reliq, deice, delta_scale=False):
        nlay, ncol = clwp.shape
        nbnd = lut["lut_extliq"].shape[0]
        tau = self.empty((nbnd, nlay, ncol)); ssa = self.empty((nbnd, nlay, ncol)); g = self.empty((nbnd, nlay, ncol))
        self._c("cloud_optics_2str_delta" if delta_scale else "cloud_optics_2str", ncol, nlay, nbnd, lut["nsize_liq"], lut["nsize_ice"],
                lut["radliq_lwr"], lut["radliq_upr"], lut["diamice_lwr"], lut["diamice_upr"],
                lut["lut_extliq"], lut["lut_ssaliq"], lut["lut_asyliq"], lut["lut_extice"], lut["lut_ssaice"], lut["lut_asyice"],
                clwp, ciwp, reliq, deice, tau, ssa, g)
        return tau, ssa, g

    def aerosol_optics(self, lut, aermr, rh, plev):
        nlay, ncol = rh.shape
        nphobic, nbnd = lut["mext_phobic"].shape
        nphilic, nhum = lut["mext_philic"].shape[:2]
        if len(aermr) != 11:
            raise ValueError("aerosol optics needs the 11 mixing ratios aermr01..aermr11")
        for m in aermr:
            if tuple(m.shape) not in ((nlay, ncol), (nlay,)):
                raise ValueError("aerosol mixing ratio must be (nlay, ncol) or (nlay,)")
        ptrs = (ctypes.c_void_p * 11)(*[m.data_ptr() for m in aermr])
        per_col = (ctypes.c_int * 11)(*[1 if m.dim() == 2 else 0 for m in aermr])
        tau = self.empty((nbnd, nlay, ncol)); ssa = self.empty((nbnd, nlay, ncol)); g = self.empty((nbnd, nlay, ncol))
        self._c("aerosol_optics", ncol, nlay, nbnd, nhum, nphobic, nphilic, ptrs, per_col, rh, plev, lut["rh_upper"],
                lut["mext_phobic"], lut["ssa_phobic"], lut["g_phobic"], lut["mext_philic"], lut["ssa_philic"], lut["g_philic"],
                tau, ssa, g)
        return tau, ssa, g

    def cloud_optics_1scl(self, lut, clwp, ciwp, reliq, deice):
        nlay, ncol = clwp.shape
        nbnd = lut["lut_extliq"].shape[0]
        tau = self.empty((nbnd, nlay, ncol))
        self._c("cloud_optics_1scl", ncol, nlay, nbnd, lut["nsize_liq"], lut["nsize_ice"],
                lut["radliq_lwr"], lut["radliq_upr"], lut["diamice_lwr"], lut["diamice_upr"],
                lut["lut_extliq"], lut["lut_ssaliq"], lut["lut_asyliq"], lut["lut_extice"], lut["lut_ssaice"], lut["lut_asyice"],
                clwp, ciwp, reliq, deice, tau)
        return tau

    def upload_lut(self, lut):
        return {k: (self.asarray(v) if isinstance(v, np.ndarray) else v) for k, v in lut.items()}

    def get_from_subset(self, ncol, nlay, nbnd, ncol_in, col_s_in, fulls, subs):
        n = len(fulls)
        PA = ctypes.c_void_p * 4
        pf = PA(*[f.data_ptr() for f in fulls] + [0]*(4-n))
        ps = PA(*[s.data_ptr() for s in subs] + [0]*(4-n))
        self._c("get_from_subset", ncol, nlay, nbnd, ncol_in, col_s_in, n, pf, ps)

    def subset_cols(self, arr, col_s, ncol_sub):
        ncol_full = arr.shape[-1]
        nrest = int(np.prod(arr.shape[:-1])) if arr.dim() > 1 else 1
        out = self.empty(tuple(arr.shape[:-1]) + (ncol_sub,))
        self._c("subset_cols", ncol_full, nrest, col_s, ncol_sub, arr, out)
        return out

    def gather_cols(self, perm, src, out):
        nrest = int(np.prod(src.shape[:-1], dtype=np.int64)) if src.dim() > 1 else 1
        self._c("gather_cols", out.shape[-1], nrest, perm, src.shape[-1], src, out)
        return out

    def gather_lastdim(self, perm, src, out):
        self._c("gather_lastdim", src.shape[1], out.shape[0], perm, src, out)
        return out
# ... 36 lines not shown
```

rte-rrtmgp-cpp_amd/pipeline.py:

```python
import contextlib
import os
import time

import numpy as np

MAX_GAUSS_PTS = 4
GAUSS_DS = np.array([
    [1./0.6096748751, 0., 0., 0.],
    [1./0.2509907356, 1/0.7908473988, 0., 0.],
    [1./0.1024922169, 1/0.4417960320, 1./0.8633751621, 0.],
    [1./0.0454586727, 1/0.2322334416, 1./0.5740198775, 1./0.903077597]])
GAUSS_WTS = np.array([
    [1., 0., 0., 0.],
    [0.2300253764, 0.7699746236, 0., 0.],
    [0.0437820218, 0.3875796738, 0.5686383044, 0.],
    [0.0092068785, 0.1285704278, 0.4323381850, 0.4298845087]])


def upload_atmosphere(be, atm):
    from .synthetic import Atmosphere
    out = {}
    for k, v in atm.__dict__.items():
        if isinstance(v, np.ndarray):
            out[k] = be.asarray(v)
# ... 165 lines not shown
    kn_grid = (nx, ny, nlay) if kn_grid is None else tuple(int(k) for k in kn_grid)

    col_dry, col_gas, _ = gas_state(be, kd_sw, atm, None, interpolate=False)
    tau = be.empty((ngpt, nlay, ncol)); ssa = be.empty((ngpt, nlay, ncol))
    g = None if getattr(be, "supports_null_g", False) else be.empty((ngpt, nlay, ncol))
    be.gas_optics_sw_direct(kd_sw, atm.p_lay, atm.t_lay, col_gas, col_dry, tau, ssa, g)
    cld = be.cloud_optics_2str(cloud_lut, atm.lwp, atm.iwp, atm.rel, atm.dei) if cloud_lut is not None else None

    F = be.np_dtype.type
    inc_dir = (be.to_numpy(kd_sw.solar_source).astype(be.np_dtype) * F(tsi[0])) * F(mu0[0])
    return tau, ssa, cld, sfc_albedo, float(mu0[0]), inc_dir, kn_grid


_STEP_ATMOSPHERE = None


def _step_atmosphere_type():
    global _STEP_ATMOSPHERE
    if _STEP_ATMOSPHERE is None:
        import dataclasses
        from .synthetic import Atmosphere
        _STEP_ATMOSPHERE = dataclasses.make_dataclass("StepAtmosphere", [(n, object, None) for n in ("mu0_lay", "altitude", "ref_altitude")],
                                                      bases=(Atmosphere,))
    return _STEP_ATMOSPHERE


_LW_FORMS = {
    "per_gpoint": ("do_broadband=False", {"n_gauss_angles > 1"}, "only the broadband LW solvers, fed by the Planck-lite chain, have that form"),
    "rescaled": ("lw_rescaling=True", set(), "the rescaled LW solver has one broadband form with one fixed angle"),
    "two_stream": ("lw_scattering=True", set(), "the two-stream LW solver has one broadband form without quadrature angles"),
    "optimal": ("optimal_angles=True", {"jacobian=True"}, "optimal angles are one angle and have no by-band form"),
    "byband": ("byband=True", set(), "no by-band Jacobians and no by-band form with several angles"),
    "angles": ("n_gauss_angles > 1", {"jacobian=True"}, None),
    "fractions": ("do_broadband=True", {"jacobian=True"}, None),
}


class ResidentSolver:

    STAGES = ("lw_gas_optics", "lw_planck", "lw_solver", "lw_reduce", "sw_gas_optics", "sw_solver", "sw_reduce")

    @staticmethod
    def resolve_options(atm, kd_lw, do_broadband=False, cloud_luts=None, byband=False, sunlit=False, jacobian=False, n_gauss_angles=1,
                        optimal_angles=False, lw_scattering=False, lw_rescaling=False, cloud_fraction=None, cloud_overlap="max_ran",
                        overlap_param=None, mu0_lay=None, altitude=None, ref_altitude=None):
        if mu0_lay is not None and altitude is not None:
            raise ValueError("ResidentSolver: mu0_lay and altitude are two ways to the same thing: give one")
        if ref_altitude is not None and altitude is None:
            raise ValueError("ResidentSolver: ref_altitude without altitude")
        for name, v, want in (("mu0_lay", mu0_lay, (atm.nlay, atm.ncol)), ("altitude", altitude, (atm.nlay, atm.ncol)),
                              ("ref_altitude", ref_altitude, (atm.ncol,)), ("cloud_fraction", cloud_fraction, (atm.nlay, atm.ncol)),
                              ("overlap_param", overlap_param, (atm.nlay-1, atm.ncol))):
            if v is not None and tuple(v.shape) != want:
                raise ValueError(f"ResidentSolver: {name} {tuple(v.shape)} is not {want}")
        if altitude is not None and bool((altitude < (0. if ref_altitude is None else ref_altitude)).any()):
            raise ValueError("ResidentSolver: an altitude lies below its column's reference altitude")
        if cloud_fraction is None:
            if overlap_param is not None:
                raise ValueError("ResidentSolver: overlap_param without cloud_fraction")
        else:
            if cloud_luts is None:
                raise ValueError("ResidentSolver: cloud_fraction needs cloud_luts (the cloud optics whose band properties are sampled)")
            if cloud_overlap not in ("max_ran", "exp_ran"):
                raise ValueError(f"ResidentSolver: cloud_overlap = {cloud_overlap!r} is not 'max_ran' or 'exp_ran'")
            if (cloud_overlap == "exp_ran") != (overlap_param is not None):
                raise ValueError("ResidentSolver: cloud_overlap='exp_ran' takes overlap_param (nlay-1, ncol), 'max_ran' takes none")
            for flag, name in ((lw_scattering, "lw_scattering=True"), (lw_rescaling, "lw_rescaling=True"), (sunlit, "sunlit=True")):
                if flag:
                    raise ValueError(f"ResidentSolver: cloud_fraction with {name} is not supported (the scattering LW solvers combine "
                                     "the band clouds themselves; the sunlit-only SW chain does not carry the column identities)")
        if not 1 <= int(n_gauss_angles) <= 4:
            raise ValueError(f"ResidentSolver: n_gauss_angles = {n_gauss_angles} is outside 1..4")
        given = [name for name, on in (("lw_rescaling=True", lw_rescaling), ("lw_scattering=True", lw_scattering),
                                       ("optimal_angles=True", optimal_angles), ("byband=True", byband),
                                       ("n_gauss_angles > 1", int(n_gauss_angles) > 1), ("jacobian=True", jacobian)) if on]
        form = "per_gpoint" if not do_broadband else next((f for f, rule in _LW_FORMS.items() if rule[0] in given), "fractions")
        chooser, admits, why = _LW_FORMS[form]
        for name in given:
            if name != chooser and name not in admits:
                raise ValueError(f"ResidentSolver: {chooser} with {name} is not supported ({why})")
        if form == "optimal" and getattr(kd_lw, "optimal_angle_fit", None) is None:
            raise ValueError("ResidentSolver: optimal_angles=True needs a LW k-distribution with optimal_angle_fit")
        return form

    def __init__(self, be, kd_lw, kd_sw, atm, do_broadband=False, overlap=False, cloud_luts=None, sort_columns=None, byband=False,
                 sunlit=False, jacobian=False, n_gauss_angles=1, optimal_angles=False, keep_secants=False, lw_scattering=False,
                 lw_rescaling=False, cloud_fraction=None, cloud_overlap="max_ran", overlap_param=None, mcica_seed=0, mcica_col_offset=0,
                 mu0_lay=None, altitude=None, ref_altitude=None, planet_radius=6.37123e6):
        import torch
        self.torch = torch
        self.lw_form = self.resolve_options(
            atm, kd_lw, do_broadband=do_broadband, cloud_luts=cloud_luts, byband=byband, sunlit=sunlit, jacobian=jacobian,
            n_gauss_angles=n_gauss_angles, optimal_angles=optimal_angles, lw_scattering=lw_scattering, lw_rescaling=lw_rescaling,
            cloud_fraction=cloud_fraction, cloud_overlap=cloud_overlap, overlap_param=overlap_param, mu0_lay=mu0_lay, altitude=altitude,
            ref_altitude=ref_altitude)
        self.be, self.kd_lw, self.kd_sw, self.atm = be, kd_lw, kd_sw, atm
        self.do_broadband, self.cloud_luts = do_broadband, cloud_luts
        self.lite = do_broadband
        self.g_zero = cloud_luts is None
        self.byband, self.jacobian, self.sunlit = bool(byband), bool(jacobian), bool(sunlit)
        self.n_gauss_angles, self.optimal_angles = int(n_gauss_angles), bool(optimal_angles)
        self.keep_secants = bool(keep_secants) and self.optimal_angles
        self.lw_scattering, self.lw_rescaling = bool(lw_scattering), bool(lw_rescaling)
        self.cloud_fraction, self.overlap_param = cloud_fraction, overlap_param
        self.mcica_seed, self.mcica_col_offset = int(mcica_seed), int(mcica_col_offset)
        self.mu0_lay, self.altitude, self.ref_altitude, self.planet_radius = mu0_lay, altitude, ref_altitude, float(planet_radius)
        if sort_columns is None:
            sort_columns = os.environ.get("RRX_SORT_COLUMNS", "auto")
        if sort_columns == "auto":
            ps = atm.p_lev[-1 if atm.top_at_1 else 0]
            nb = (atm.ncol // 256) * 256
            if nb >= 256:
                blk = ps[:nb].reshape(-1, 256)
                sort_columns = bool((((blk.max(dim=1).values - blk.min(dim=1).values) / blk.mean(dim=1)) > 0.2).any().item())
            else:
                sort_columns = False
        self.sort_columns = bool(sort_columns) and str(sort_columns) != "0"
        pad16 = bool(int(os.environ.get("RRX_PAD_COLUMNS", "1"))) and atm.ncol > 16
        self.npad = (16 - atm.ncol % 16) if (pad16 and atm.ncol % 16 != 0) else 0
        self.ncol_caller = atm.ncol
        self.perm = None
        if self.sort_columns or self.npad:
            self.refresh_column_order()
        self.overlap = overlap
        self.streams = [torch.cuda.Stream(device=be.device), torch.cuda.Stream(device=be.device)] if overlap else None

        ncol, nlay = atm.ncol + self.npad, atm.nlay
        ng_l, ng_s = kd_lw.ngpt, kd_sw.ngpt
        e = be.empty
        self.col_dry = e((nlay, ncol))
        self.col_dry2 = None
        if do_broadband:
            self.lw = dict(tau=e((ng_l, nlay, ncol)), pfrac=e((ng_l, nlay, ncol)), blay=e((kd_lw.nbnd, nlay, ncol)),
                           blev=e((kd_lw.nbnd, nlay+1, ncol)), sfc_src=e((ng_l, ncol)), sfc_src_jac=e((ng_l, ncol)))
        else:
            self.lw = dict(tau=e((ng_l, nlay, ncol)), lay_src=e((ng_l, nlay, ncol)), lev_src=e((ng_l, nlay+1, ncol)),
                           sfc_src=e((ng_l, ncol)), sfc_src_jac=e((ng_l, ncol)))
        self.sw = dict(tau=e((ng_s, nlay, ncol)), ssa=e((ng_s, nlay, ncol)), g=e((ng_s, nlay, ncol)))
        if not do_broadband:
            self.lw.update(gpt_up=e((ng_l, nlay+1, ncol)), gpt_dn=e((ng_l, nlay+1, ncol)))
            self.sw.update(gpt_up=e((ng_s, nlay+1, ncol)), gpt_dn=e((ng_s, nlay+1, ncol)), gpt_dir=e((ng_s, nlay+1, ncol)))
        self.fluxes = e((7, nlay+1, atm.ncol))
        self.fluxes_sorted = e((7, nlay+1, ncol)) if self.perm is not None else None
        self.lw_flux_up_jac = e((nlay+1, atm.ncol)) if self.jacobian else None
        self.jac_sorted = e((nlay+1, ncol)) if (self.jacobian and self.perm is not None) else None
        self.bnd_lw = self.bnd_sw = self.bnd_lw_sorted = self.bnd_sw_sorted = None
        self.bnd_fluxes = None
        if self.byband:
            self.bnd_lw = e((3, kd_lw.nbnd, nlay+1, atm.ncol)); self.bnd_sw = e((4, kd_sw.nbnd, nlay+1, atm.ncol))
            if self.perm is not None:
                self.bnd_lw_sorted = e((3, kd_lw.nbnd, nlay+1, ncol)); self.bnd_sw_sorted = e((4, kd_sw.nbnd, nlay+1, ncol))
            self.bnd_fluxes = dict(lw_up=self.bnd_lw[0], lw_dn=self.bnd_lw[1], lw_net=self.bnd_lw[2],
                                   sw_up=self.bnd_sw[0], sw_dn=self.bnd_sw[1], sw_dir=self.bnd_sw[2], sw_net=self.bnd_sw[3])
        own = self.perm is None
        self._F = tuple(self.fluxes if own else self.fluxes_sorted)
        self._BL = tuple(self.bnd_lw if own else self.bnd_lw_sorted) if self.byband else None
        self._BS = tuple(self.bnd_sw if own else self.bnd_sw_sorted) if self.byband else None
        if self.sunlit:
            self.sun_pad = 16 if pad16 else 1
            nmax = -(-atm.ncol // self.sun_pad) * self.sun_pad
            assert nmax <= ncol
            self.sun_perm = be.int_empty((nmax,))
            self.sun_count = be.int_empty((1,))
            self.sun_count_host = torch.empty((1,), dtype=torch.int32, pin_memory=True)
            self.sun_event = torch.cuda.Event()
            self.sun_wait_ms = 0.0
            self.sun_in = {}
            for k in self._SW_FIELDS:
                v = getattr(self._step_atmosphere(), k, None)
                if v is not None and (cloud_luts is not None or k not in ("lwp", "iwp", "rel", "dei")):
                    self.sun_in[k] = e(tuple(v.shape[:-1]) + (ncol,) if self._COLUMN_FIELDS[k] < 0 else (ncol,) + tuple(v.shape[1:]))
            self.sun_vmr = {n: e((nlay, ncol)) for n, t in atm.vmr.items() if hasattr(t, "dim") and t.dim() == 2}
            self.sun_fluxes = e((4, nlay+1, ncol))
            self.sun_bnd = e((4, kd_sw.nbnd, nlay+1, ncol)) if self.byband else None
        self.weights = be.asarray(np.ascontiguousarray(GAUSS_WTS[self.n_gauss_angles-1, :self.n_gauss_angles]))
        self.gauss_Ds = be.asarray(GAUSS_DS)
        self.secants = e((self.n_gauss_angles, ng_l, ncol))
        self.optimal_fit = be.optimal_fit_abi(kd_lw) if self.optimal_angles else None
        self.lw_secants = e((ng_l, ncol)) if self.keep_secants else None
        self.sfc_emis_gpt = e((ng_l, ncol)); self.alb_dir = e((ng_s, ncol)); self.alb_dif = e((ng_s, ncol))
        self.mu0_lay_step = e((nlay, ncol)) if self.altitude is not None else None
        self.events = self._rec = None



    def enable_stage_events(self, nsteps):
        ev = self.torch.cuda.Event
        self.events = [{s: (ev(enable_timing=True), ev(enable_timing=True)) for s in self.STAGES} for _ in range(nsteps)]
        self._istep = 0

    def stage_ms(self):
        out = {s: [] for s in self.STAGES}
        for rec in self.events[:self._istep]:
            for s, (a, b) in rec.items():
                out[s].append(a.elapsed_time(b))
        return {s: float(np.mean(v)) for s, v in out.items() if v}

    _COLUMN_FIELDS = {"p_lay": -1, "p_lev": -1, "t_lay": -1, "t_lev": -1, "t_sfc": 0, "mu0": 0, "tsi_scaling": 0,
                      "emis_sfc": 0, "sfc_alb_dir": 0, "sfc_alb_dif": 0, "lwp": -1, "iwp": -1, "rel": -1, "dei": -1, "rh": -1,
                      "mu0_lay": -1, "altitude": -1, "ref_altitude": 0}

    _SW_FIELDS = ("p_lay", "p_lev", "t_lay", "mu0", "tsi_scaling", "sfc_alb_dir", "sfc_alb_dif", "lwp", "iwp", "rel", "dei",
                  "mu0_lay", "altitude", "ref_altitude")

    def _step_atmosphere(self):
        if self.mu0_lay is None and self.altitude is None:
            return self.atm
        return _step_atmosphere_type()(**self.atm.__dict__, mu0_lay=self.mu0_lay, altitude=self.altitude, ref_altitude=self.ref_altitude)

    @staticmethod
    def _cols(t, n):
        lead = tuple(t.shape[:-1])
        return t.view(-1)[:int(np.prod(lead, dtype=np.int64))*n].view(lead + (n,))

    @staticmethod
    def _rows(t, n):
        rest = tuple(t.shape[1:])
        return t.view(-1)[:int(np.prod(rest, dtype=np.int64))*n].view((n,) + rest)

    def _sunlit_atmosphere(self, n_out):
        be, a, perm = self.be, self._step_atmosphere(), self.sun_perm
        out = dict(a.__dict__)
        out["ncol"] = n_out
        for k, buf in self.sun_in.items():
            v = getattr(a, k, None)
            if v is None:
                continue
            if self._COLUMN_FIELDS[k] < 0 or v.dim() == 1:
                out[k] = be.gather_cols(perm, v, self._cols(buf, n_out) if self._COLUMN_FIELDS[k] < 0 else buf[:n_out])
            else:
                out[k] = be.gather_lastdim(perm, v, self._rows(buf, n_out))
        out["vmr"] = {n: (be.gather_cols(perm, t, self._cols(self.sun_vmr[n], n_out)) if n in self.sun_vmr else t)
                      for n, t in a.vmr.items()}
        return type(a)(**out)

    def refresh_column_order(self):
        torch = self.torch
        a = self.atm
        if self.sort_columns:
            perm = torch.argsort(a.p_lev[-1 if a.top_at_1 else 0])
        else:
            perm = torch.arange(a.ncol, device=a.p_lev.device)
        if self.npad:
            perm = torch.cat([perm, perm[-1:].expand(self.npad)])
        self.perm = perm.contiguous()
        self.perm_i32 = self.perm.to(torch.int32)

    def _gathered_atmosphere(self):
        a, perm = self._step_atmosphere(), self.perm
        out = {}
        for k, v in a.__dict__.items():
            if k == "ncol":
                out[k] = int(perm.numel())
            elif k in self._COLUMN_FIELDS and v is not None:
                out[k] = v.index_select(v.dim() - 1 if self._COLUMN_FIELDS[k] < 0 else 0, perm)
            elif isinstance(v, dict):
                out[k] = {n: (t.index_select(1, perm) if (hasattr(t, "dim") and t.dim() == 2) else t) for n, t in v.items()}
            else:
                out[k] = v
        return type(a)(**out)

    def _mark(self, stage, end=False):
        if self._rec is not None:
            self._rec[stage][1 if end else 0].record(self.torch.cuda.current_stream(self.be.device))

    def _chain_stream(self, ichain, main):
        if not self.overlap:
            return contextlib.nullcontext()
        self.streams[ichain].wait_stream(main)
        return self.torch.cuda.stream(self.streams[ichain])

    def step(self):
        be, atm = self.be, self._step_atmosphere()
        perm = self.perm
        if perm is not None:
            atm = self._gathered_atmosphere()
        if self.overlap and self.col_dry2 is None:
            self.col_dry2 = be.empty(tuple(self.col_dry.shape))
        self._rec = None
        if self.events is not None and self._istep < len(self.events):
            self._rec = self.events[self._istep]
            self._istep += 1
        mcica = None
        if self.cloud_fraction is not None:
            cfrac, alpha, col_id = self.cloud_fraction, self.overlap_param, None
            if perm is not None:
                cfrac = cfrac.index_select(1, perm)
                alpha = None if alpha is None else alpha.index_select(1, perm)
                col_id = self.perm_i32 + self.mcica_col_offset
            mcica = (cfrac, alpha, col_id)
        F, BL, BS = self._F, self._BL, self._BS
        J = self.lw_flux_up_jac if perm is None else self.jac_sorted
        main = self.torch.cuda.current_stream(be.device)
        if self.sunlit:
            n = self.ncol_caller
            be.sunlit_columns(self.atm.mu0, None if perm is None else self.perm_i32[:n], self.sun_pad, perm=self.sun_perm, count=self.sun_count)
            self.sun_count_host.copy_(self.sun_count, non_blocking=True)
            self.sun_event.record(main)
        with self._chain_stream(0, main):
            self._lw_chain(atm, self.col_dry, self.lw, F, J, BL, mcica)
        sw_day = False
        with self._chain_stream(1, main):
            self._mark("sw_gas_optics")
            col_dry = self.col_dry2 if self.overlap else self.col_dry
            if self.sunlit:
                t0 = time.perf_counter()
                self.sun_event.synchronize()
                self.sun_wait_ms += (time.perf_counter() - t0) * 1e3
                n_day = int(self.sun_count_host[0])
                sw_day = n_day < self.ncol_caller
            if sw_day:
                n_out = -(-n_day // self.sun_pad) * self.sun_pad
                self._sw_chain(self._sunlit_atmosphere(n_out) if n_day else None, self._cols(col_dry, n_out),
                               {k: self._cols(v, n_out) for k, v in self.sw.items()}, self._cols(self.alb_dir, n_out),
                               self._cols(self.alb_dif, n_out), self._cols(self.sun_fluxes, n_out),
                               self._cols(self.sun_bnd, n_out) if self.byband else None, None, n_day=n_day)
            else:
                self._sw_chain(atm, col_dry, self.sw, self.alb_dir, self.alb_dif, F[3:], BS, mcica)
        if self.overlap:
            main.wait_stream(self.streams[0]); main.wait_stream(self.streams[1])
        if perm is not None:
            n = self.ncol_caller
            nf = 3 if sw_day else 7
            self.fluxes[:nf].index_copy_(2, perm[:n], self.fluxes_sorted[:nf, :, :n])
            if self.jacobian:
                self.lw_flux_up_jac.index_copy_(1, perm[:n], J[:, :n])
            if self.byband:
                self.bnd_lw.index_copy_(3, perm[:n], self.bnd_lw_sorted[..., :n])
                if not sw_day:
                    self.bnd_sw.index_copy_(3, perm[:n], self.bnd_sw_sorted[..., :n])
        return self.fluxes

    def _lw_chain(self, atm, col_dry, buf, F, J, BL, mcica):
        be, kd, mark = self.be, self.kd_lw, self._mark
        form = self.lw_form
        mark("lw_gas_optics")
        be.get_col_dry(atm.vmr["h2o"], atm.p_lev, out=col_dry)
        col_gas = be.fill_gases(kd, atm.vmr, col_dry)
        tc = cld = None
        if self.cloud_luts is not None and form in ("two_stream", "rescaled"):
            cld = be.cloud_optics_2str(self.cloud_luts[0], atm.lwp, atm.iwp, atm.rel, atm.dei)
        elif self.cloud_luts is not None:
            tc = be.cloud_optics_1scl(self.cloud_luts[0], atm.lwp, atm.iwp, atm.rel, atm.dei)
        fused = tc if mcica is None else None
        if form == "per_gpoint":
            be.gas_optics_lw_direct(kd, atm.p_lay, atm.t_lay, col_gas, buf["tau"], by_band=fused)
        else:
            be.gas_optics_lw_fractions(kd, atm.p_lay, atm.t_lay, atm.t_lev, atm.t_sfc, _sfc_lay(atm), col_gas, buf["tau"], out=buf,
                                       by_band=fused)
        if tc is not None and mcica is not None:
            be.mcica_increment_1scalar(buf["tau"], tc, kd.band_lims_gpt, mcica[0], mcica[1], self.mcica_seed, 0, mcica[2], self.mcica_col_offset)
        mark("lw_gas_optics", True)
        mark("lw_planck")
        if form == "per_gpoint":
            be.planck_source_direct(kd, atm.p_lay, atm.t_lay, atm.t_lev, atm.t_sfc, _sfc_lay(atm), col_gas, out=buf)
        mark("lw_planck", True)
        mark("lw_solver")
        if form not in ("optimal", "two_stream"):
            be.lw_secants_array(atm.ncol, kd.ngpt, self.n_gauss_angles, MAX_GAUSS_PTS, self.gauss_Ds, out=self.secants)
        be.expand_and_transpose(kd.band_lims_gpt, atm.emis_sfc, kd.ngpt, out=self.sfc_emis_gpt)
        top, sec, wts, tau, emis = atm.top_at_1, self.secants, self.weights, buf["tau"], self.sfc_emis_gpt
        if form == "rescaled":
            be.lw_solver_noscat_fractions_rescaled(top, kd, sec, wts, tau, buf, emis, cloud=cld, flux_up=F[0], flux_dn=F[1])
        elif form == "two_stream":
            be.lw_solver_2stream_fractions(top, kd, tau, buf, emis, cloud=cld, flux_up=F[0], flux_dn=F[1])
        elif form == "optimal":
            be.lw_solver_noscat_fractions_optimal(top, kd, wts, tau, buf, emis, fit=self.optimal_fit, flux_up=F[0], flux_dn=F[1],
                                                  flux_up_jac=J, jacobian=self.jacobian, secants_out=self.lw_secants)
        elif form == "byband":
            be.lw_solver_noscat_fractions_byband(top, kd, sec, wts, tau, buf, emis,
                                                 out=dict(bnd_flux_up=BL[0], bnd_flux_dn=BL[1], bnd_flux_net=BL[2], flux_up=F[0], flux_dn=F[1]))
        elif form == "angles":
            be.lw_solver_noscat_fractions_angles(top, kd, sec, wts, tau, buf, emis, flux_up=F[0], flux_dn=F[1], flux_up_jac=J,
                                                 jacobian=self.jacobian)
        elif form == "fractions" and self.jacobian:
            be.lw_solver_noscat_fractions_jac(top, kd, sec, wts, tau, buf, emis, flux_up=F[0], flux_dn=F[1], flux_up_jac=J)
        elif form == "fractions":
            be.lw_solver_noscat_fractions(top, kd, sec, wts, tau, buf, emis, flux_up=F[0], flux_dn=F[1])
        else:
            be.lw_solver_noscat(top, sec, wts, tau, buf["lay_src"], buf["lev_src"], emis, buf["sfc_src"],
                                out=dict(flux_up=buf["gpt_up"], flux_dn=buf["gpt_dn"]))
        mark("lw_solver", True)
        mark("lw_reduce")
        if form == "per_gpoint":
            be.sum_broadband(buf["gpt_up"], out=F[0]); be.sum_broadband(buf["gpt_dn"], out=F[1])
        be.net_broadband_precalc(F[1], F[0], out=F[2])
        mark("lw_reduce", True)

    def _sw_chain(self, atm, col_dry, buf, alb_dir, alb_dif, F, BS, mcica, n_day=None):
        be, kd, mark = self.be, self.kd_sw, self._mark
        if n_day == 0:
            mark("sw_gas_optics", True); mark("sw_solver"); mark("sw_solver", True); mark("sw_reduce")
            self._sunlit_scatter(0, 0, BS)
            mark("sw_reduce", True)
            return
        be.get_col_dry(atm.vmr["h2o"], atm.p_lev, out=col_dry)
        col_gas = be.fill_gases(kd, atm.vmr, col_dry)
        gbuf = None if (self.g_zero and self.do_broadband) else buf["g"]
        cld = None
        if self.cloud_luts is not None:
            cld = be.cloud_optics_2str(self.cloud_luts[1], atm.lwp, atm.iwp, atm.rel, atm.dei, delta_scale=True)
        be.gas_optics_sw_direct(kd, atm.p_lay, atm.t_lay, col_gas, col_dry, buf["tau"], buf["ssa"], gbuf, by_band=cld if mcica is None else None)
        toa = be.toa_source(atm.ncol, kd.solar_source, atm.tsi_scaling)
        if cld is not None and mcica is not None:
            be.mcica_increment_2stream(buf["tau"], buf["ssa"], gbuf, *cld, kd.band_lims_gpt, mcica[0], mcica[1], self.mcica_seed, 1, mcica[2],
                                       self.mcica_col_offset)
        mark("sw_gas_optics", True)
        mark("sw_solver")
        be.expand_and_transpose(kd.band_lims_gpt, atm.sfc_alb_dir, kd.ngpt, out=alb_dir)
        be.expand_and_transpose(kd.band_lims_gpt, atm.sfc_alb_dif, kd.ngpt, out=alb_dif)
        mu0_lay = getattr(atm, "mu0_lay", None)
        if self.altitude is not None:
            mu0_lay = be.zenith_angle_spherical_correction(atm.mu0, atm.altitude, atm.ref_altitude, self.planet_radius,
                                                           out=self._cols(self.mu0_lay_step, atm.ncol))
        if self.do_broadband:
            out = dict(flux_up=F[0], flux_dn=F[1], flux_dir=F[2])
        else:
            out = dict(flux_up=buf["gpt_up"], flux_dn=buf["gpt_dn"], flux_dir=buf["gpt_dir"])
        if self.byband:
            out.update(bnd_flux_up=BS[0], bnd_flux_dn=BS[1], bnd_flux_dir=BS[2], bnd_flux_net=BS[3])
        top, tau, ssa = atm.top_at_1, buf["tau"], buf["ssa"]
        if mu0_lay is not None and self.byband:
            be.sw_solver_2stream_byband_mu0lay(top, tau, ssa, gbuf, mu0_lay, alb_dir, alb_dif, toa, kd.band_lims_gpt, out=out)
        elif mu0_lay is not None:
            be.sw_solver_2stream_mu0lay(top, tau, ssa, gbuf, mu0_lay, alb_dir, alb_dif, toa, do_broadband=self.do_broadband, out=out)
        elif self.byband:
            be.sw_solver_2stream_byband(top, tau, ssa, gbuf, atm.mu0, alb_dir, alb_dif, toa, kd.band_lims_gpt, out=out)
        else:
            be.sw_solver_2stream(top, tau, ssa, gbuf, atm.mu0, alb_dir, alb_dif, toa, do_broadband=self.do_broadband, out=out)
        mark("sw_solver", True)
        mark("sw_reduce")
        if not self.do_broadband:
            be.sum_broadband(buf["gpt_up"], out=F[0]); be.sum_broadband(buf["gpt_dn"], out=F[1]); be.sum_broadband(buf["gpt_dir"], out=F[2])
        be.net_broadband_precalc(F[1], F[0], out=F[3])
        if n_day is not None:
            self._sunlit_scatter(n_day, atm.ncol, BS)
        mark("sw_reduce", True)

    def _sunlit_scatter(self, n_day, n_out, BSd):
        be = self.be
        be.scatter_cols_fill(n_day, self.sun_perm, self._cols(self.sun_fluxes, n_out), self.fluxes[3:7])
        if self.byband:
            be.scatter_cols_fill(n_day, self.sun_perm, BSd, self.bnd_sw)
```

Baseline: 1.434 million columns/s.

## Fuse per-step input prep into one kernel and pair LW/SW net-flux kernels

Merges col_dry computation, gas column filling for LW and SW, surface emissivity/albedo expansion, TOA source and LW secant fill into one multi-task step_inputs kernel that runs once per step. It also pairs the LW and SW net-flux subtractions into one launch and moves the gas-window todo-header zeroing from a memset into the table-build kernel. The goal is fewer small kernel launches and less duplicated col_dry/col_gas work. In exchange it adds buffer plumbing and a dependency between the LW and SW chains, and it changes how LW and SW can overlap.

```diff
diff --git a/include/rrx_hip.h b/include/rrx_hip.h
--- a/include/rrx_hip.h
+++ b/include/rrx_hip.h
@@ -343,6 +343,9 @@
 int rrx_sum_broadband##SFX(int ncol, int nlev, int ngpt, const F* gpt_flux, F* flux, void* stream); \
 int rrx_net_broadband_precalc##SFX(int ncol, int nlev, const F* flux_dn, const F* flux_up, F* flux_net, void* stream); \
  \
+int rrx_net_broadband_pair##SFX(int ncol, int nlev, const F* flux_dn_a, const F* flux_up_a, F* flux_net_a, \
+        const F* flux_dn_b, const F* flux_up_b, F* flux_net_b, void* stream); \
+ \
 int rrx_heating_rate##SFX(int ncol, int nlay, F g_over_cp, const F* flux_net, const F* plev, F* heating_rate, void* stream); \
  \
 int rrx_sum_byband##SFX(int ncol, int nlev, int ngpt, int nbnd, const int* band_lims, const F* gpt_flux, F* bnd_flux, void* stream); \
@@ -365,6 +368,15 @@
 int rrx_scaling_to_subset##SFX(int ncol, int ngpt, F* toa_src, const F* tsi_scaling, void* stream); \
  \
 int rrx_toa_source##SFX(int ncol, int ngpt, F* toa_src, const F* solar_source, const F* tsi_scaling, void* stream); \
+ \
+int rrx_step_inputs##SFX(int ncol, int nlay, const F* vmr_h2o, const F* p_lev, const F* col_dry_in, F* col_dry, \
+        int ngas_a, const F* const* vmr_a, const int* dim1_a, const int* dim2_a, F* col_gas_a, \
+        int ngas_b, const F* const* vmr_b, const int* dim1_b, const int* dim2_b, F* col_gas_b, \
+        int nbnd_0, const int* band_lims_gpt_0, const F* arr_in_0, int ngpt_0, F* arr_out_0, \
+        int nbnd_1, const int* band_lims_gpt_1, const F* arr_in_1, int ngpt_1, F* arr_out_1, \
+        int nbnd_2, const int* band_lims_gpt_2, const F* arr_in_2, int ngpt_2, F* arr_out_2, \
+        int ngpt_toa, const F* solar_source, const F* tsi_scaling, F* toa_src, \
+        int ngpt_sec, int n_gauss_quad, int max_gauss_pts, const F* gauss_Ds, F* secants, void* stream); \
  \
 int rrx_aerosol_optics##SFX(int ncol, int nlay, int nbnd, int nhum, int nphobic, int nphilic, const F* const* aermr, const int* aermr_per_column, \
         const F* rh, const F* plev, const F* rh_upper, const F* mext_phobic, const F* ssa_phobic, const F* g_phobic, \
diff --git a/rte-rrtmgp-cpp_amd/csrc/rrx_common.h b/rte-rrtmgp-cpp_amd/csrc/rrx_common.h
--- a/rte-rrtmgp-cpp_amd/csrc/rrx_common.h
+++ b/rte-rrtmgp-cpp_amd/csrc/rrx_common.h
@@ -214,6 +214,12 @@
         constexpr int NXCD = 8;
         const int per = n / NXCD, whole = per*NXCD;
         return (w < whole) ? (w % NXCD)*per + w / NXCD : w;
+    }
+
+    template<typename F>
+    __device__ __forceinline__ F lw_secant_value(const F* __restrict__ gauss_Ds, const int imu, const int n_gauss_quad, const int max_gauss_pts)
+    {
+        return gauss_Ds[imu + (n_gauss_quad-1)*max_gauss_pts];
     }
 
     inline int ceil_div(const long long a, const long long b) { return int((a + b - 1) / b); }
diff --git a/rte-rrtmgp-cpp_amd/csrc/rrx_gas_optics.hip b/rte-rrtmgp-cpp_amd/csrc/rrx_gas_optics.hip
--- a/rte-rrtmgp-cpp_amd/csrc/rrx_gas_optics.hip
+++ b/rte-rrtmgp-cpp_amd/csrc/rrx_gas_optics.hip
@@ -1216,9 +1216,10 @@
         const int* __restrict__ idx_minor_lower, const int* __restrict__ idx_minor_upper,
         const int* __restrict__ idx_minor_scaling_lower, const int* __restrict__ idx_minor_scaling_upper,
         const int* __restrict__ kminor_start_lower, const int* __restrict__ kminor_start_upper,
-        int* __restrict__ tbl)
+        int* __restrict__ tbl, int* __restrict__ todo_header)
 {
     extern __shared__ int lds_int[];
+    if (threadIdx.x < 9) todo_header[threadIdx.x] = 0;
     const int nmax = max(nminorlower, nminorupper);
     const GasWindowTables T{ngpt, nmax, ncmax};
     constexpr int LIT = GasWindowTables::LIT;
@@ -2164,7 +2165,6 @@
     p.nblk = int(p.grid.x)*int(p.grid.y);
     p.nz = gas_window_parts(p.nblk, nchunk);
     p.todo = scratch.get<int>(size_t(9) + size_t(p.nblk)*p.nz) + 8;
-    if (hipMemsetAsync(p.todo - 8, 0, 9*sizeof(int), st) != hipSuccess) throw std::runtime_error("memset failed");
     const GasWindowTables T{k.ngpt, nmax, p.ncmax};
     const int* lims = ia.cld_tau != nullptr ? ia.cld_lims : nullptr;
     p.tbl = gas_window_tables(st, k.gpoint_flavor, k.ngpt, k.nminorlower, k.nminorupper, p.ncmax, nlist, (pf ? 1 : 0) + (lims != nullptr ? 2 : 0));
@@ -2173,7 +2173,7 @@
             k.minor_limits_gpt_lower, k.minor_limits_gpt_upper,
             k.minor_scales_with_density_lower, k.minor_scales_with_density_upper, k.scale_by_complement_lower, k.scale_by_complement_upper,
             k.idx_minor_lower, k.idx_minor_upper, k.idx_minor_scaling_lower, k.idx_minor_scaling_upper,
-            k.kminor_start_lower, k.kminor_start_upper, p.tbl);
+            k.kminor_start_lower, k.kminor_start_upper, p.tbl, p.todo - 8);
     return p;
 }
 
diff --git a/rte-rrtmgp-cpp_amd/csrc/rrx_misc.hip b/rte-rrtmgp-cpp_amd/csrc/rrx_misc.hip
--- a/rte-rrtmgp-cpp_amd/csrc/rrx_misc.hip
+++ b/rte-rrtmgp-cpp_amd/csrc/rrx_misc.hip
@@ -196,9 +196,23 @@
 }
 
 template<typename F>
+__device__ __forceinline__ void net_range(const size_t n, const F* __restrict__ dn, const F* __restrict__ up, F* __restrict__ net)
+{
+    RRX_GRID_STRIDE(i, n) net[i] = dn[i] - up[i];
+}
+
+template<typename F>
 __global__ void net_kernel(const size_t n, const F* __restrict__ dn, const F* __restrict__ up, F* __restrict__ net)
 {
-    RRX_GRID_STRIDE(i, n) net[i] = dn[i] - up[i];
+    net_range(n, dn, up, net);
+}
+
+template<typename F>
+__global__ void net_pair_kernel(const size_t n, const F* __restrict__ dn_a, const F* __restrict__ up_a, F* __restrict__ net_a,
+                                const F* __restrict__ dn_b, const F* __restrict__ up_b, F* __restrict__ net_b)
+{
+    if (blockIdx.y == 0) net_range(n, dn_a, up_a, net_a);
+    else                 net_range(n, dn_b, up_b, net_b);
 }
 
 template<typename F, bool NET>
@@ -259,48 +273,57 @@
 template<typename F> struct GasTable { const F* vmr[RRX_MAX_GASES]; int dim1[RRX_MAX_GASES], dim2[RRX_MAX_GASES]; };
 
 template<typename F>
+__device__ __forceinline__ void fill_gases_cell(const size_t i, const size_t ncl, const int ncol, const int ngas, const GasTable<F>& gt,
+                                                F* __restrict__ col_gas, const F cd)
+{
+    col_gas[i] = cd;
+    for (int igas=0; igas<ngas; ++igas)
+    {
+        const F* __restrict__ src = gt.vmr[igas];
+        const F v = (gt.dim1[igas] == 1 && gt.dim2[igas] == 1) ? src[0] : (gt.dim1[igas] == 1 ? src[i / ncol] : src[i]);
+        col_gas[i + size_t(igas+1)*ncl] = v * cd;
+    }
+}
+
+template<typename F>
 __global__ void fill_gases_all_kernel(const int ncol, const int nlay, const int ngas, const GasTable<F> gt,
                                       F* __restrict__ col_gas, const F* __restrict__ col_dry)
 {
     const size_t ncl = size_t(ncol)*nlay;
-    RRX_GRID_STRIDE(i, ncl)
-    {
-        const F cd = col_dry[i];
-        col_gas[i] = cd;
-        for (int igas=0; igas<ngas; ++igas)
-        {
-            const F* __restrict__ src = gt.vmr[igas];
-            const F v = (gt.dim1[igas] == 1 && gt.dim2[igas] == 1) ? src[0] : (gt.dim1[igas] == 1 ? src[i / ncol] : src[i]);
-            col_gas[i + size_t(igas+1)*ncl] = v * cd;
-        }
-    }
-}
-
-template<typename F>
-__global__ void col_dry_kernel(const int ncol, const int nlay, const F* __restrict__ vmr_h2o, const F* __restrict__ plev, F* __restrict__ col_dry)
+    RRX_GRID_STRIDE(i, ncl) fill_gases_cell(i, ncl, ncol, ngas, gt, col_gas, col_dry[i]);
+}
+
+template<typename F>
+__device__ __forceinline__ F col_dry_cell(const F plev_a, const F plev_b, const F h)
 {
     constexpr F g0 = 9.80665;
     constexpr F avogad = 6.02214076e23;
     constexpr F m_dry = 0.028964;
     constexpr F m_h2o = 0.018016;
+    const F delta_plev = abs(plev_a - plev_b);
+    const F m_air = (m_dry + m_h2o * h) / (F(1.) + h);
+    F cd = F(10.) * delta_plev * avogad / (F(1000.)*m_air*F(100.)*g0);
+    cd /= (F(1.) + h);
+    return cd;
+}
+
+template<typename F>
+__global__ void col_dry_kernel(const int ncol, const int nlay, const F* __restrict__ vmr_h2o, const F* __restrict__ plev, F* __restrict__ col_dry)
+{
     const size_t ncl = size_t(ncol)*nlay;
     RRX_GRID_STRIDE(i, ncl)
     {
-        const F delta_plev = abs(plev[i] - plev[i + ncol]);
-        const F h = vmr_h2o[i];
-        const F m_air = (m_dry + m_h2o * h) / (F(1.) + h);
-        F cd = F(10.) * delta_plev * avogad / (F(1000.)*m_air*F(100.)*g0);
-        cd /= (F(1.) + h);
-        col_dry[i] = cd;
-    }
-}
-
-template<typename F>
-__global__ void expand_and_transpose_kernel(const int ncol, const int nbnd, const int* __restrict__ limits, const F* __restrict__ in, F* __restrict__ out)
-{
-    const int ibnd = blockIdx.y;
+        const F plev_a = plev[i], plev_b = plev[i + ncol];
+        col_dry[i] = col_dry_cell(plev_a, plev_b, vmr_h2o[i]);
+    }
+}
+
+template<typename F>
+__device__ __forceinline__ void expand_band(const int ncol, const int nbnd, const int ibnd, const int bx, const int nbx,
+                                            const int* __restrict__ limits, const F* __restrict__ in, F* __restrict__ out)
+{
     const int g0 = limits[2*ibnd]-1, g1 = limits[2*ibnd+1];
-    RRX_GRID_STRIDE(icol, size_t(ncol))
+    for (size_t icol = size_t(bx)*blockDim.x + threadIdx.x; icol < size_t(ncol); icol += size_t(nbx)*blockDim.x)
     {
         const F v = in[ibnd + icol*nbnd];
         for (int ig=g0; ig<g1; ++ig) out[icol + size_t(ig)*ncol] = v;
@@ -308,10 +331,24 @@
 }
 
 template<typename F>
+__global__ void expand_and_transpose_kernel(const int ncol, const int nbnd, const int* __restrict__ limits, const F* __restrict__ in, F* __restrict__ out)
+{
+    expand_band(ncol, nbnd, int(blockIdx.y), int(blockIdx.x), int(gridDim.x), limits, in, out);
+}
+
+template<typename F, bool SCALED>
+__device__ __forceinline__ void toa_row(const int ncol, const int igpt, const int bx, const int nbx,
+                                        F* __restrict__ out, const F* __restrict__ src, const F* __restrict__ fac)
+{
+    const F v = src[igpt];
+    for (int icol = bx*blockDim.x + threadIdx.x; icol < ncol; icol += nbx*blockDim.x)
+        out[icol + size_t(igpt)*ncol] = SCALED ? v * fac[icol] : v;
+}
+
+template<typename F>
 __global__ void spread_col_kernel(const int ncol, const int ngpt, F* __restrict__ out, const F* __restrict__ src)
 {
-    const F v = src[blockIdx.y];
-    for (int icol = blockIdx.x*blockDim.x + threadIdx.x; icol < ncol; icol += gridDim.x*blockDim.x) out[icol + size_t(blockIdx.y)*ncol] = v;
+    toa_row<F,false>(ncol, int(blockIdx.y), int(blockIdx.x), int(gridDim.x), out, src, nullptr);
 }
 
 template<typename F>
@@ -323,8 +360,66 @@
 template<typename F>
 __global__ void toa_source_kernel(const int ncol, const int ngpt, F* __restrict__ out, const F* __restrict__ src, const F* __restrict__ fac)
 {
-    const F v = src[blockIdx.y];
-    for (int icol = blockIdx.x*blockDim.x + threadIdx.x; icol < ncol; icol += gridDim.x*blockDim.x) out[icol + size_t(blockIdx.y)*ncol] = v * fac[icol];
+    toa_row<F,true>(ncol, int(blockIdx.y), int(blockIdx.x), int(gridDim.x), out, src, fac);
+}
+
+template<typename F> struct ExpandTask { const int* limits; const F* in; F* out; int nbnd, nbx; };
+template<typename F> struct StepInputs
+{
+    int ncol, nlay;
+    const F* vmr_h2o; const F* plev; const F* col_dry_in; F* col_dry;
+    int ngas[2]; F* col_gas[2]; GasTable<F> gt[2];
+    ExpandTask<F> ex[3];
+    int toa_nbx; const F* solar_source; const F* tsi_scaling; F* toa_src;
+    int sec_nbx, sec_ngpt, n_gauss_quad, max_gauss_pts; const F* gauss_Ds; F* secants;
+    unsigned end[6];
+};
+
+template<typename F>
+__global__ void __launch_bounds__(256) step_inputs_kernel(const StepInputs<F> a)
+{
+    const unsigned b = blockIdx.x;
+    if (b < a.end[0])
+    {
+        const size_t ncl = size_t(a.ncol)*a.nlay;
+        for (size_t i = size_t(b)*256 + threadIdx.x; i < ncl; i += size_t(a.end[0])*256)
+        {
+            F cd;
+            if (a.vmr_h2o != nullptr)
+            {
+                const F plev_a = a.plev[i], plev_b = a.plev[i + a.ncol];
+                cd = col_dry_cell(plev_a, plev_b, a.vmr_h2o[i]);
+                if (a.col_dry != nullptr) a.col_dry[i] = cd;
+            }
+            else
+                cd = a.col_dry_in[i];
+            if (a.col_gas[0] != nullptr) fill_gases_cell(i, ncl, a.ncol, a.ngas[0], a.gt[0], a.col_gas[0], cd);
+            if (a.col_gas[1] != nullptr) fill_gases_cell(i, ncl, a.ncol, a.ngas[1], a.gt[1], a.col_gas[1], cd);
+        }
+        return;
+    }
+    #pragma unroll
+    for (int t=0; t<3; ++t)
+        if (b < a.end[1+t])
+        {
+            const ExpandTask<F>& e = a.ex[t];
+            const int lb = int(b - a.end[t]);
+            expand_band(a.ncol, e.nbnd, lb / e.nbx, lb % e.nbx, e.nbx, e.limits, e.in, e.out);
+            return;
+        }
+    if (b < a.end[4])
+    {
+        const int lb = int(b - a.end[3]);
+        if (a.tsi_scaling != nullptr) toa_row<F,true>(a.ncol, lb / a.toa_nbx, lb % a.toa_nbx, a.toa_nbx, a.toa_src, a.solar_source, a.tsi_scaling);
+        else                          toa_row<F,false>(a.ncol, lb / a.toa_nbx, lb % a.toa_nbx, a.toa_nbx, a.toa_src, a.solar_source, nullptr);
+        return;
+    }
+    const int lb = int(b - a.end[4]);
+    const int imu = lb / a.sec_nbx;
+    const F v = lw_secant_value(a.gauss_Ds, imu, a.n_gauss_quad, a.max_gauss_pts);
+    const size_t n = size_t(a.ncol)*a.sec_ngpt;
+    F* __restrict__ out = a.secants + size_t(imu)*n;
+    for (size_t i = size_t(lb % a.sec_nbx)*256 + threadIdx.x; i < n; i += size_t(a.sec_nbx)*256) out[i] = v;
 }
 
 template<typename F>
@@ -602,6 +697,58 @@
 int rrx_net_broadband_precalc##SFX(int ncol, int nlev, const F* flux_dn, const F* flux_up, F* flux_net, void* stream) \
 { RRX_TRY const size_t n = size_t(ncol)*nlev; \
   net_kernel<F><<<grid1d(n), 256, 0, ST>>>(n, flux_dn, flux_up, flux_net); RRX_CATCH("rrx_net_broadband_precalc") } \
+int rrx_net_broadband_pair##SFX(int ncol, int nlev, const F* flux_dn_a, const F* flux_up_a, F* flux_net_a, \
+        const F* flux_dn_b, const F* flux_up_b, F* flux_net_b, void* stream) \
+{ RRX_TRY const size_t n = extent({ncol, nlev}); \
+  if (flux_net_a == nullptr) throw std::runtime_error("no first net flux"); \
+  if (n == 0) return 0; \
+  net_pair_kernel<F><<<dim3(grid1d(n), flux_net_b != nullptr ? 2 : 1), 256, 0, ST>>>(n, flux_dn_a, flux_up_a, flux_net_a, \
+      flux_dn_b, flux_up_b, flux_net_b); RRX_CATCH("rrx_net_broadband_pair") } \
+int rrx_step_inputs##SFX(int ncol, int nlay, const F* vmr_h2o, const F* p_lev, const F* col_dry_in, F* col_dry, \
+        int ngas_a, const F* const* vmr_a, const int* dim1_a, const int* dim2_a, F* col_gas_a, \
+        int ngas_b, const F* const* vmr_b, const int* dim1_b, const int* dim2_b, F* col_gas_b, \
+        int nbnd_0, const int* band_lims_gpt_0, const F* arr_in_0, int ngpt_0, F* arr_out_0, \
+        int nbnd_1, const int* band_lims_gpt_1, const F* arr_in_1, int ngpt_1, F* arr_out_1, \
+        int nbnd_2, const int* band_lims_gpt_2, const F* arr_in_2, int ngpt_2, F* arr_out_2, \
+        int ngpt_toa, const F* solar_source, const F* tsi_scaling, F* toa_src, \
+        int ngpt_sec, int n_gauss_quad, int max_gauss_pts, const F* gauss_Ds, F* secants, void* stream) \
+{ RRX_TRY StepInputs<F> a{}; \
+  if (ngas_a < 0 || ngas_a > RRX_MAX_GASES || ngas_b < 0 || ngas_b > RRX_MAX_GASES) throw std::runtime_error("more gases than a table of rrx_step_inputs takes"); \
+  const size_t ncl = extent({ncol, nlay}); \
+  a.ncol = ncol; a.nlay = nlay; \
+  const bool computes = vmr_h2o != nullptr || p_lev != nullptr; \
+  if (computes && (vmr_h2o == nullptr || p_lev == nullptr)) throw std::runtime_error("col_dry is computed from vmr_h2o and p_lev: one of them is missing"); \
+  if (computes && col_dry_in != nullptr) throw std::runtime_error("col_dry is either computed (vmr_h2o, p_lev) or given (col_dry_in): give one"); \
+  const bool cells = ncl > 0 && (col_dry != nullptr || col_gas_a != nullptr || col_gas_b != nullptr); \
+  if (cells && !computes && col_dry != nullptr) throw std::runtime_error("the col_dry output needs vmr_h2o and p_lev"); \
+  if (cells && !computes && col_dry_in == nullptr) throw std::runtime_error("the col_gas outputs need vmr_h2o and p_lev, or col_dry_in"); \
+  unsigned nb = 0; \
+  if (cells) \
+  { a.vmr_h2o = vmr_h2o; a.plev = p_lev; a.col_dry_in = col_dry_in; a.col_dry = col_dry; \
+    const int ng[2] = {ngas_a, ngas_b}; const F* const* vm[2] = {vmr_a, vmr_b}; const int* d1[2] = {dim1_a, dim1_b}; \
+    const int* d2[2] = {dim2_a, dim2_b}; F* cg[2] = {col_gas_a, col_gas_b}; \
+    for (int t=0; t<2; ++t) \
+    { a.col_gas[t] = cg[t]; a.ngas[t] = cg[t] != nullptr ? ng[t] : 0; \
+      for (int i=0; i<a.ngas[t]; ++i) { a.gt[t].vmr[i] = vm[t][i]; a.gt[t].dim1[i] = d1[t][i]; a.gt[t].dim2[i] = d2[t][i]; } } \
+    nb += unsigned(grid1d(ncl)); } \
+  a.end[0] = nb; \
+  { const int nbnd[3] = {nbnd_0, nbnd_1, nbnd_2}; const int ngpt[3] = {ngpt_0, ngpt_1, ngpt_2}; \
+    const int* lims[3] = {band_lims_gpt_0, band_lims_gpt_1, band_lims_gpt_2}; \
+    const F* in[3] = {arr_in_0, arr_in_1, arr_in_2}; F* out[3] = {arr_out_0, arr_out_1, arr_out_2}; \
+    for (int t=0; t<3; ++t) \
+    { if (out[t] != nullptr && extent({ncol, nbnd[t], ngpt[t]}) > 0) \
+      { a.ex[t] = ExpandTask<F>{lims[t], in[t], out[t], nbnd[t], std::min(grid1d(ncol), 1024)}; nb += unsigned(a.ex[t].nbx)*unsigned(nbnd[t]); } \
+      a.end[1+t] = nb; } } \
+  if (toa_src != nullptr && extent({ncol, ngpt_toa}) > 0) \
+  { a.toa_nbx = std::min(ceil_div(ncol, 256), 64); a.solar_source = solar_source; a.tsi_scaling = tsi_scaling; a.toa_src = toa_src; \
+    nb += unsigned(a.toa_nbx)*unsigned(ngpt_toa); } \
+  a.end[4] = nb; \
+  if (secants != nullptr && extent({ncol, ngpt_sec, n_gauss_quad}) > 0) \
+  { a.sec_nbx = grid1d(size_t(ncol)*ngpt_sec); a.sec_ngpt = ngpt_sec; a.n_gauss_quad = n_gauss_quad; a.max_gauss_pts = max_gauss_pts; \
+    a.gauss_Ds = gauss_Ds; a.secants = secants; nb += unsigned(a.sec_nbx)*unsigned(n_gauss_quad); } \
+  a.end[5] = nb; \
+  if (nb == 0) return 0; \
+  step_inputs_kernel<F><<<nb, 256, 0, ST>>>(a); RRX_CATCH("rrx_step_inputs") } \
 int rrx_heating_rate##SFX(int ncol, int nlay, F g_over_cp, const F* flux_net, const F* plev, F* heating_rate, void* stream) \
 { RRX_TRY const size_t n = extent({ncol, nlay}); if (n == 0) return 0; \
   heating_rate_kernel<F><<<grid1d(n), 256, 0, ST>>>(n, ncol, g_over_cp, flux_net, plev, heating_rate); RRX_CATCH("rrx_heating_rate") } \
diff --git a/rte-rrtmgp-cpp_amd/csrc/rrx_solver_lw.hip b/rte-rrtmgp-cpp_amd/csrc/rrx_solver_lw.hip
--- a/rte-rrtmgp-cpp_amd/csrc/rrx_solver_lw.hip
+++ b/rte-rrtmgp-cpp_amd/csrc/rrx_solver_lw.hip
@@ -712,7 +712,7 @@
     for (size_t i = size_t(blockIdx.x)*blockDim.x + threadIdx.x; i < n; i += size_t(gridDim.x)*blockDim.x)
     {
         const int imu = int(i / (size_t(ncol)*ngpt));
-        secants[i] = gauss_Ds[imu + (n_gauss_quad-1)*max_gauss_pts];
+        secants[i] = lw_secant_value(gauss_Ds, imu, n_gauss_quad, max_gauss_pts);
     }
 }
 
diff --git a/rte-rrtmgp-cpp_amd/hip_kernels.py b/rte-rrtmgp-cpp_amd/hip_kernels.py
--- a/rte-rrtmgp-cpp_amd/hip_kernels.py
+++ b/rte-rrtmgp-cpp_amd/hip_kernels.py
@@ -609,6 +609,10 @@
         self._c("net_broadband_precalc", ncol, nlev, flux_dn, flux_up, out)
         return out
 
+    def net_broadband_pair(self, dn_a, up_a, net_a, dn_b=None, up_b=None, net_b=None):
+        nlev, ncol = dn_a.shape
+        self._c("net_broadband_pair", ncol, nlev, dn_a, up_a, net_a, dn_b, up_b, net_b)
+
     def heating_rate(self, flux_net, plev, g_over_cp=9.80665/1004.64):
         nlev, ncol = flux_net.shape
         out = self.empty((nlev-1, ncol))
@@ -661,6 +665,53 @@
         for i, (v, (d1, d2)) in enumerate(zip(vs, dims), start=1):
             self._c("fill_gases", ncol, nlay, d1, d2, kd.ngas, i, vmr, v, col_gas, col_dry)
         return col_gas
+
+    def gas_table(self, gas_names, vmr_by_name, nlay, ncol):
+        vs =[vmr_by_name[name] for name in gas_names]
+        dims = [self._vmr_dims(name, v, nlay, ncol) for name, v in zip(gas_names, vs)]
+        n = len(vs)
+        return (n, (ctypes.c_void_p * n)(*[v.data_ptr() for v in vs]), (ctypes.c_int * n)(*[d[0] for d in dims]),
+                (ctypes.c_int * n)(*[d[1] for d in dims]), vs)
+
+    def step_inputs(self, ncol, nlay, vmr_h2o=None, p_lev=None, col_dry_in=None, col_dry=None, gases=(), expansions=(), toa=None,
+                    secants=None):
+        if len(gases) > 2 or len(expansions) > 3:
+            raise ValueError("step_inputs takes at most two gas tables and three expansions")
+        args = [ncol, nlay, vmr_h2o, p_lev, col_dry_in, col_dry]
+        keep = []
+        for k in range(2):
+            if k < len(gases):
+                names, vmr, col_gas = gases[k]
+                n, ptrs, d1, d2, vs = self.gas_table(names, vmr, nlay, ncol)
+                if tuple(col_gas.shape) != (n+1, nlay, ncol):
+                    raise ValueError(f"step_inputs: col_gas {tuple(col_gas.shape)} is not {(n+1, nlay, ncol)}")
+                keep.append(vs)
+                args += [n, ptrs, d1, d2, col_gas]
+            else:
+                args += [0, None, None, None, None]
+        for k in range(3):
+            if k < len(expansions):
+                lims, arr_in, out = expansions[k]
+                if tuple(arr_in.shape) != (ncol, lims.shape[0]) or out.shape[1] != ncol:
+                    raise ValueError(f"step_inputs: expansion {k} of {tuple(arr_in.shape)} into {tuple(out.shape)} with {ncol} columns")
+                args += [lims.shape[0], lims, arr_in, out.shape[0], out]
+            else:
+                args += [0, None, None, 0, None]
+        if toa is not None:
+            src, tsi, out = toa
+            if tuple(out.shape) != (src.shape[0], ncol):
+                raise ValueError(f"step_inputs: toa_src {tuple(out.shape)} is not {(src.shape[0], ncol)}")
+            args += [src.shape[0], src, tsi, out]
+        else:
+            args += [0, None, None, None]
+        if secants is not None:
+            n_quad, max_pts, gauss_Ds, out = secants
+            if out.shape[0] != n_quad or out.shape[2] != ncol:
+                raise ValueError(f"step_inputs: secants {tuple(out.shape)} with {n_quad} angles and {ncol} columns")
+            args += [out.shape[1], n_quad, max_pts, gauss_Ds, out]
+        else:
+            args += [0, 0, 0, None, None]
+        self._c("step_inputs", *args)
 
     def expand_and_transpose(self, band_lims, arr_in, ngpt, out=None):
         ncol, nbnd = arr_in.shape
diff --git a/rte-rrtmgp-cpp_amd/pipeline.py b/rte-rrtmgp-cpp_amd/pipeline.py
--- a/rte-rrtmgp-cpp_amd/pipeline.py
+++ b/rte-rrtmgp-cpp_amd/pipeline.py
@@ -271,6 +271,10 @@
         if form == "optimal" and getattr(kd_lw, "optimal_angle_fit", None) is None:
             raise ValueError("ResidentSolver: optimal_angles=True needs a LW k-distribution with optimal_angle_fit")
         return form
+
+    @staticmethod
+    def shares_col_gas(kd_lw, kd_sw):
+        return list(kd_lw.gas_names) == list(kd_sw.gas_names)
 
     def __init__(self, be, kd_lw, kd_sw, atm, do_broadband=False, overlap=False, cloud_luts=None, sort_columns=None, byband=False,
                  sunlit=False, jacobian=False, n_gauss_angles=1, optimal_angles=False, keep_secants=False, lw_scattering=False,
@@ -318,7 +322,6 @@
         ng_l, ng_s = kd_lw.ngpt, kd_sw.ngpt
         e = be.empty
         self.col_dry = e((nlay, ncol))
-        self.col_dry2 = None
         if do_broadband:
             self.lw = dict(tau=e((ng_l, nlay, ncol)), pfrac=e((ng_l, nlay, ncol)), blay=e((kd_lw.nbnd, nlay, ncol)),
                            blev=e((kd_lw.nbnd, nlay+1, ncol)), sfc_src=e((ng_l, ncol)), sfc_src_jac=e((ng_l, ncol)))
@@ -369,6 +372,15 @@
         self.lw_secants = e((ng_l, ncol)) if self.keep_secants else None
         self.sfc_emis_gpt = e((ng_l, ncol)); self.alb_dir = e((ng_s, ncol)); self.alb_dif = e((ng_s, ncol))
         self.mu0_lay_step = e((nlay, ncol)) if self.altitude is not None else None
+        for kd in (kd_lw, kd_sw):
+            if len(kd.gas_names) > 32:
+                raise ValueError(f"ResidentSolver: a k-distribution with {len(kd.gas_names)} gases (rrx_step_inputs takes 32 per table)")
+        self.col_gas_lw = e((len(kd_lw.gas_names)+1, nlay, ncol))
+        self.sw_own_inputs = self.sunlit
+        self.one_col_gas = self.shares_col_gas(kd_lw, kd_sw) and not self.sw_own_inputs
+        self.col_gas_sw = self.col_gas_lw if self.one_col_gas else e((len(kd_sw.gas_names)+1, nlay, ncol))
+        self.sun_col_dry = e((nlay, ncol)) if self.sunlit else None
+        self.toa = e((ng_s, ncol))
         self.events = self._rec = None
 
 
@@ -464,8 +476,6 @@
         perm = self.perm
         if perm is not None:
             atm = self._gathered_atmosphere()
-        if self.overlap and self.col_dry2 is None:
-            self.col_dry2 = be.empty(tuple(self.col_dry.shape))
         self._rec = None
         if self.events is not None and self._istep < len(self.events):
             self._rec = self.events[self._istep]
@@ -486,12 +496,25 @@
             be.sunlit_columns(self.atm.mu0, None if perm is None else self.perm_i32[:n], self.sun_pad, perm=self.sun_perm, count=self.sun_count)
             self.sun_count_host.copy_(self.sun_count, non_blocking=True)
             self.sun_event.record(main)
+        kd_lw, kd_sw = self.kd_lw, self.kd_sw
+        self._mark("lw_gas_optics")
+        gases = [(kd_lw.gas_names, atm.vmr, self.col_gas_lw)]
+        expansions = [(kd_lw.band_lims_gpt, atm.emis_sfc, self.sfc_emis_gpt)]
+        if not self.sw_own_inputs:
+            if not self.one_col_gas:
+                gases.append((kd_sw.gas_names, atm.vmr, self.col_gas_sw))
+            expansions += [(kd_sw.band_lims_gpt, atm.sfc_alb_dir, self.alb_dir), (kd_sw.band_lims_gpt, atm.sfc_alb_dif, self.alb_dif)]
+        be.step_inputs(atm.ncol, atm.nlay, vmr_h2o=atm.vmr["h2o"], p_lev=atm.p_lev, col_dry=self.col_dry, gases=gases,
+                       expansions=expansions, toa=None if self.sw_own_inputs else (kd_sw.solar_source, atm.tsi_scaling, self.toa),
+                       secants=None if self.lw_form in ("optimal", "two_stream")
+                       else (self.n_gauss_angles, MAX_GAUSS_PTS, self.gauss_Ds, self.secants))
+        lw_net = (F[1], F[0], F[2]) if not (self.overlap or self.sunlit) else None
         with self._chain_stream(0, main):
-            self._lw_chain(atm, self.col_dry, self.lw, F, J, BL, mcica)
+            self._lw_chain(atm, self.col_gas_lw, self.lw, F, J, BL, mcica, own_net=lw_net is None)
         sw_day = False
         with self._chain_stream(1, main):
             self._mark("sw_gas_optics")
-            col_dry = self.col_dry2 if self.overlap else self.col_dry
+            col_dry = self.col_dry
             if self.sunlit:
                 t0 = time.perf_counter()
                 self.sun_event.synchronize()
@@ -500,12 +523,14 @@
                 sw_day = n_day < self.ncol_caller
             if sw_day:
                 n_out = -(-n_day // self.sun_pad) * self.sun_pad
-                self._sw_chain(self._sunlit_atmosphere(n_out) if n_day else None, self._cols(col_dry, n_out),
+                self._sw_chain(self._sunlit_atmosphere(n_out) if n_day else None, self._cols(self.sun_col_dry, n_out),
+                               self._cols(self.col_gas_sw, n_out), self._cols(self.toa, n_out),
                                {k: self._cols(v, n_out) for k, v in self.sw.items()}, self._cols(self.alb_dir, n_out),
                                self._cols(self.alb_dif, n_out), self._cols(self.sun_fluxes, n_out),
-                               self._cols(self.sun_bnd, n_out) if self.byband else None, None, n_day=n_day)
+                               self._cols(self.sun_bnd, n_out) if self.byband else None, None, n_day=n_day, own_inputs="compute")
             else:
-                self._sw_chain(atm, col_dry, self.sw, self.alb_dir, self.alb_dif, F[3:], BS, mcica)
+                self._sw_chain(atm, col_dry, self.col_gas_sw, self.toa, self.sw, self.alb_dir, self.alb_dif, F[3:], BS, mcica,
+                               own_inputs="col_dry" if self.sw_own_inputs else None, lw_net=lw_net)
         if self.overlap:
             main.wait_stream(self.streams[0]); main.wait_stream(self.streams[1])
         if perm is not None:
@@ -520,12 +545,9 @@
                     self.bnd_sw.index_copy_(3, perm[:n], self.bnd_sw_sorted[..., :n])
         return self.fluxes
 
-    def _lw_chain(self, atm, col_dry, buf, F, J, BL, mcica):
+    def _lw_chain(self, atm, col_gas, buf, F, J, BL, mcica, own_net=True):
         be, kd, mark = self.be, self.kd_lw, self._mark
         form = self.lw_form
-        mark("lw_gas_optics")
-        be.get_col_dry(atm.vmr["h2o"], atm.p_lev, out=col_dry)
-        col_gas = be.fill_gases(kd, atm.vmr, col_dry)
         tc = cld = None
         if self.cloud_luts is not None and form in ("two_stream", "rescaled"):
             cld = be.cloud_optics_2str(self.cloud_luts[0], atm.lwp, atm.iwp, atm.rel, atm.dei)
@@ -545,9 +567,6 @@
             be.planck_source_direct(kd, atm.p_lay, atm.t_lay, atm.t_lev, atm.t_sfc, _sfc_lay(atm), col_gas, out=buf)
         mark("lw_planck", True)
         mark("lw_solver")
-        if form not in ("optimal", "two_stream"):
-            be.lw_secants_array(atm.ncol, kd.ngpt, self.n_gauss_angles, MAX_GAUSS_PTS, self.gauss_Ds, out=self.secants)
-        be.expand_and_transpose(kd.band_lims_gpt, atm.emis_sfc, kd.ngpt, out=self.sfc_emis_gpt)
         top, sec, wts, tau, emis = atm.top_at_1, self.secants, self.weights, buf["tau"], self.sfc_emis_gpt
         if form == "rescaled":
             be.lw_solver_noscat_fractions_rescaled(top, kd, sec, wts, tau, buf, emis, cloud=cld, flux_up=F[0], flux_dn=F[1])
@@ -573,31 +592,34 @@
         mark("lw_reduce")
         if form == "per_gpoint":
             be.sum_broadband(buf["gpt_up"], out=F[0]); be.sum_broadband(buf["gpt_dn"], out=F[1])
-        be.net_broadband_precalc(F[1], F[0], out=F[2])
+        if own_net:
+            be.net_broadband_pair(F[1], F[0], F[2])
         mark("lw_reduce", True)
 
-    def _sw_chain(self, atm, col_dry, buf, alb_dir, alb_dif, F, BS, mcica, n_day=None):
+    def _sw_chain(self, atm, col_dry, col_gas, toa, buf, alb_dir, alb_dif, F, BS, mcica, n_day=None, own_inputs=None, lw_net=None):
         be, kd, mark = self.be, self.kd_sw, self._mark
         if n_day == 0:
             mark("sw_gas_optics", True); mark("sw_solver"); mark("sw_solver", True); mark("sw_reduce")
             self._sunlit_scatter(0, 0, BS)
             mark("sw_reduce", True)
             return
-        be.get_col_dry(atm.vmr["h2o"], atm.p_lev, out=col_dry)
-        col_gas = be.fill_gases(kd, atm.vmr, col_dry)
+        if own_inputs is not None:
+            compute = own_inputs == "compute"
+            be.step_inputs(atm.ncol, atm.nlay, vmr_h2o=atm.vmr["h2o"] if compute else None, p_lev=atm.p_lev if compute else None,
+                           col_dry_in=None if compute else col_dry, col_dry=col_dry if compute else None,
+                           gases=[(kd.gas_names, atm.vmr, col_gas)],
+                           expansions=[(kd.band_lims_gpt, atm.sfc_alb_dir, alb_dir), (kd.band_lims_gpt, atm.sfc_alb_dif, alb_dif)],
+                           toa=(kd.solar_source, atm.tsi_scaling, toa))
         gbuf = None if (self.g_zero and self.do_broadband) else buf["g"]
         cld = None
         if self.cloud_luts is not None:
             cld = be.cloud_optics_2str(self.cloud_luts[1], atm.lwp, atm.iwp, atm.rel, atm.dei, delta_scale=True)
         be.gas_optics_sw_direct(kd, atm.p_lay, atm.t_lay, col_gas, col_dry, buf["tau"], buf["ssa"], gbuf, by_band=cld if mcica is None else None)
-        toa = be.toa_source(atm.ncol, kd.solar_source, atm.tsi_scaling)
         if cld is not None and mcica is not None:
             be.mcica_increment_2stream(buf["tau"], buf["ssa"], gbuf, *cld, kd.band_lims_gpt, mcica[0], mcica[1], self.mcica_seed, 1, mcica[2],
                                        self.mcica_col_offset)
         mark("sw_gas_optics", True)
         mark("sw_solver")
-        be.expand_and_transpose(kd.band_lims_gpt, atm.sfc_alb_dir, kd.ngpt, out=alb_dir)
-        be.expand_and_transpose(kd.band_lims_gpt, atm.sfc_alb_dif, kd.ngpt, out=alb_dif)
         mu0_lay = getattr(atm, "mu0_lay", None)
         if self.altitude is not None:
             mu0_lay = be.zenith_angle_spherical_correction(atm.mu0, atm.altitude, atm.ref_altitude, self.planet_radius,
@@ -621,7 +643,7 @@
         mark("sw_reduce")
         if not self.do_broadband:
             be.sum_broadband(buf["gpt_up"], out=F[0]); be.sum_broadband(buf["gpt_dn"], out=F[1]); be.sum_broadband(buf["gpt_dir"], out=F[2])
-        be.net_broadband_precalc(F[1], F[0], out=F[3])
+        be.net_broadband_pair(F[1], F[0], F[3], *(lw_net or ()))
         if n_day is not None:
             self._sunlit_scatter(n_day, atm.ncol, BS)
         mark("sw_reduce", True)
```

New measurement: 1.432 million columns/s. Within noise of the previous version (-0.1%).
